# google-research/multinerf

Hardware: AMD Instinct MI355X
Metric: train_rays_per_sec (higher is better)
Workload: dtype bf16 MFMA inputs / fp32 accumulate, fp32 everywhere else

## Files before the change

### include/mnerf.h

```cpp
#ifndef MNERF_H_
#define MNERF_H_

#include <stdint.h>

#ifdef __cplusplus
extern "C" {
#endif

typedef enum {
  MNR_OK = 0,
  MNR_ERR_INVALID_ARGUMENT = -1,
  MNR_ERR_HIP = -2,
  MNR_ERR_UNSUPPORTED = -3
} mnr_status;

const char* mnr_last_error(void);
int mnr_abi_version(void);
int mnr_device_info(int device, int* cu_count, int* lds_bytes_per_cu, char* arch_name, int arch_name_len);

typedef enum { MNR_RAYDIST_IDENTITY = 0, MNR_RAYDIST_RECIPROCAL = 1, MNR_RAYDIST_PIECEWISE = 2,
               MNR_RAYDIST_LOG = 3, MNR_RAYDIST_EXP = 4, MNR_RAYDIST_SQRT = 5, MNR_RAYDIST_SQUARE = 6 } mnr_raydist;

typedef struct {
  int n_prev;
// ... 59 lines not shown

int mnr_viewdir_enc_fill(int64_t B, int n, const float* viewdirs, int deg_view,
                         uint16_t* dst, int ld, int col0, int col_end, void* stream);

typedef enum { MNR_CAM_PERSPECTIVE = 0, MNR_CAM_FISHEYE = 1 } mnr_camtype;
int mnr_pixels_to_rays(int64_t B, const int32_t* pix_x_int, const int32_t* pix_y_int, const int32_t* cam_idx,
                       int num_cams, const float* pixtocams, const float* camtoworlds, const float* distortion6,
                       const float* pixtocam_ndc, int camtype, float* origins, float* directions, float* viewdirs,
                       float* radii, float* imageplane, void* stream);

int mnr_spherical_rays(int H, int W, const float* camtoworld, float* origins, float* directions, float* viewdirs,
                       float* radii, float* imageplane, void* stream);

int mnr_glo_fill(int64_t B, int n, int G, const float* table, const int32_t* cam_idx, int num_embeddings,
                 uint16_t* dst, int ld, int col0, void* stream);
int mnr_glo_bwd(int64_t B, int n, int G, const float* g_a, const float* g_b, const int32_t* cam_idx,
                int num_embeddings, float* grad_table, void* stream);

typedef struct {
  const uint16_t* A1; int lda1; int K1;
  const uint16_t* A2; int lda2; int K2;
  const uint16_t* Bt; int ldb;
  int64_t M;
  int N;
  const float* bias; int n_bias;
  int relu;
  const uint16_t* mask; int ldmask;
  uint16_t* Cb; int ldcb; int nb;
  float* Cf; int ldcf; int f0; int nf;
  uint8_t* mask_bits_out; int ld_bits_out;
  const uint8_t* mask_bits_in; int ld_bits_in;
  int64_t bits_row_mod;
  int a1_layout; int c_layout;
  const uint16_t* vcol; float* vcol_out; const float* vcol_bias;
  int walk_descending;
  int max_wgs;
} mnr_gemm_nt_args;
#define MNR_LAYOUT_ROWMAJOR 0
#define MNR_LAYOUT_PANEL 1

int mnr_gemm_nt_bf16(const mnr_gemm_nt_args* args, void* stream);

#define MNR_CHAIN_MAX_DEPTH 8
typedef struct {
  int64_t M;
  int W;
  int depth;
  const uint16_t* feat;
  int ld_feat; int K0;
  const uint16_t* Bt[MNR_CHAIN_MAX_DEPTH];
  int ldb[MNR_CHAIN_MAX_DEPTH];
  const float* bias[MNR_CHAIN_MAX_DEPTH];
  const uint16_t* w_head;
  const float* b_head;
  float* head_out;
  uint16_t* acts[MNR_CHAIN_MAX_DEPTH];
  uint8_t* bits[MNR_CHAIN_MAX_DEPTH];
  int skip_layer;
} mnr_mlp_chain_fwd_args;
int mnr_mlp_chain_fwd(const mnr_mlp_chain_fwd_args* args, void* stream);

#define MNR_CHAIN_IPE_GROUP_COLS 192
typedef struct {
  mnr_ipe_cfg cfg;
  int n;
  const float* tdist;
  const float* origins; const float* directions; const float* radii; const float* basis;
} mnr_chain_ipe_args;
int mnr_mlp_chain_fwd_ipe(const mnr_mlp_chain_fwd_args* chain, const mnr_chain_ipe_args* ipe, void* stream);

typedef struct {
  int64_t M; int W; int depth;
  const float* g_head;
  const float* w_head;
  const uint8_t* bits[MNR_CHAIN_MAX_DEPTH];
  const uint16_t* Bw[MNR_CHAIN_MAX_DEPTH];
  int ldb[MNR_CHAIN_MAX_DEPTH];
  uint16_t* dY[MNR_CHAIN_MAX_DEPTH];
  const uint16_t* dY_in;
} mnr_mlp_chain_bwd_args;
int mnr_mlp_chain_bwd(const mnr_mlp_chain_bwd_args* args, void* stream);

typedef struct {
  const uint16_t* A; int lda; int K;
  const uint16_t* B; int ldb; int N;
  int64_t M;
  float* C; int ldc;
  int k_valid, n_valid;
  float* bias_out; int bias_n_valid;
  const uint16_t* gcol; float* gcol_out;
  int a_layout, b_layout;
  int m_interleave, max_wgs;
  const float* rank1_g; const float* rank1_w; const uint8_t* rank1_bits; int ld_rank1_bits;
} mnr_gemm_tn_args;

int mnr_gemm_tn_bf16(const mnr_gemm_tn_args* args, void* stream);

int mnr_colsum_bf16(const uint16_t* X, int ld, int64_t M, int n_valid, float* out, void* stream);

typedef struct {
  int64_t src_off; int rows_in; int cols_out;
  int64_t dst_off; int ld; int row0; int col0; int transpose;
} mnr_pack_desc;
int mnr_pack_weights_bf16(const float* params, const mnr_pack_desc* descs_device, int n_desc,
                          int max_elems, uint16_t* dst, void* stream);

int mnr_scatter_add_f32(const float* src, int ld_src, int row0, int col0, int rows, int cols,
                        float* dst, int ld_dst, void* stream);

int mnr_cast_f32_to_bf16(const float* src, int ld_src, int64_t M, int n, uint16_t* dst, int ld_dst,
                         int col0, void* stream);

int mnr_act_fwd_bf16(int kind, int64_t n, const uint16_t* z, uint16_t* a, void* stream);
int mnr_act_bwd_bf16(int kind, int64_t n, const uint16_t* z, uint16_t* d, void* stream);
int mnr_act_tangent_fwd_bf16(int kind, int64_t n, const uint16_t* z, const uint16_t* U, uint16_t* T, void* stream);
int mnr_act_tangent_bwd_bf16(int kind, int64_t n, const uint16_t* z, const uint16_t* U, uint16_t* G, uint16_t* extra, void* stream);

int mnr_add_noise_bf16(int64_t M, int cols, uint16_t* X, int ld, const float* noise, float scale, void* stream);

int mnr_small_head_bwd(int64_t M, int K, int C, const uint16_t* H, int ldh, const float* g,
                       const float* W, uint16_t* dX, int lddx, int apply_relu_mask,
                       float* dW, float* db,
                       const uint8_t* mask_bits ,
                       int ld_bits, int64_t bits_row_mod,
                       float* scratch ,
                       int64_t scratch_floats, void* stream);

typedef enum { MNR_ACT_SIGMOID = 0, MNR_ACT_SAFE_EXP = 1, MNR_ACT_SOFTPLUS = 2, MNR_ACT_EXP = 3,
               MNR_ACT_RELU = 4 } mnr_act;

typedef struct {
  int n;
  int opaque_background;
  int density_act;
  float density_bias;
  float density_noise_std;
  int has_rgb;
  int rgb_act;
  float rgb_premultiplier, rgb_bias, rgb_padding;
  int bg_mode;
  float bg_value;
} mnr_composite_cfg;

int mnr_composite_fwd(const mnr_composite_cfg* cfg, int64_t B, const float* raw_density,
                      const float* density_noise, const float* raw_rgb, const float* tdist,
                      const float* dirs, const float* bg, const float* exposure_scale,
                      float* density, float* rgb, float* weights, float* rgb_out, float* acc,
                      void* stream);

int mnr_composite_bwd(const mnr_composite_cfg* cfg, int64_t B, const float* raw_density,
                      const float* density_noise, const float* raw_rgb, const float* tdist,
                      const float* dirs, const float* bg, const float* exposure_scale,
                      const float* weights, const float* g_rgb_out, const float* g_weights,
                      float* g_raw_density, uint16_t* g_raw_density_bf16, int ld_bf16,
                      float* g_raw_rgb, float* g_exposure_scale , void* stream);

typedef struct {
  mnr_composite_cfg cfg;
  int64_t B, B_valid;
  const float* raw_density; const float* density_noise; const float* raw_rgb; const float* tdist; const float* dirs;
  const float* bg; const float* exposure_scale; const float* weights;
  const float* g_rgb_out;
  const float* g_weights;
  float* g_raw_density; uint16_t* g_raw_density_bf16; int ld_bf16; float* g_raw_rgb; float* g_exposure_scale;
  int data_loss_type; float charb_padding; float data_loss_mult;
  const float* rgb_out; const float* gt; const float* lossmult; int lm_c; const float* denom; float* data_stats;
  int wloss_mode; float wloss_mult; const float* sdist; int n_ref; const float* t_ref; const float* w_ref; float* wloss_stat;
  float* g_x;
} mnr_level_bwd_args;
int mnr_level_bwd(const mnr_level_bwd_args* args, void* stream);

typedef struct {
  int64_t B, B_valid; int n;
  const float* sdist; const float* near; const float* far; int raydist_fn;
  const float* g_x; const float* raw_density; const float* density_noise; float density_noise_std; float density_bias;
  int density_act; const float* dirs;
  const float* g_t0; const float* g_t1;
  float distortion_mult; const float* weights;
  const float* g_sdist_in;
  float* g_sdist;
} mnr_sdist_bwd_args;
int mnr_sdist_bwd(const mnr_sdist_bwd_args* args, void* stream);

int mnr_exposure_scale(int64_t B, const float* exposure_values, const int32_t* exposure_idx,
                       const float* offsets, float* out, void* stream);
int mnr_exposure_scale_bwd(int64_t B_valid, const float* exposure_values, const int32_t* exposure_idx,
                           const float* g_scale, float* g_offsets, void* stream);

int mnr_render_extras(int64_t B, int n, const float* weights, const float* tdist, const float* t_far,
                      float* out, void* stream);

typedef struct {
  int T; int lmax;
  const int32_t* m; const int32_t* l;
  const float* sigma;
  const float* mat;
} mnr_ide_tables;

#define MNR_REF_PRED_NORMALS    1
#define MNR_REF_DENSITY_NORMALS 2
#define MNR_REF_REFLECT         4
#define MNR_REF_IDE             8
#define MNR_REF_N_DOT_V        16
#define MNR_REF_ROUGHNESS      32

int mnr_ref_head_fwd(int64_t M, int n, const float* small, const float* raw_grad, const float* viewdirs,
                     const mnr_ide_tables* tabs, int features, int deg_view, float roughness_bias, uint16_t* vi, int ldvi,
                     int col0, int col_end, float* normals_out, float* normals_pred_out, float* roughness_out, void* stream);
int mnr_ref_head_bwd(int64_t M, int n, const float* small, const float* raw_grad, const float* viewdirs,
                     const mnr_ide_tables* tabs, int features, int deg_view, float roughness_bias, const uint16_t* dvi_a,
                     const uint16_t* dvi_b, int lddvi, int col0, const float* g_npred, const float* g_n,
                     uint16_t* dhb, int lddhb, int col_gp, int col_rough, float* g_raw_grad, void* stream);
int mnr_add_cols_bf16(int64_t M, int cols, const uint16_t* a, int lda, const uint16_t* b, int ldb, uint16_t* dst,
                      int lddst, void* stream);
int mnr_ref_color_fwd(int64_t M, const float* raw_rgb, const float* small, float rgb_premultiplier, float rgb_bias,
                      float rgb_padding, int use_tint, float* rgb_out, void* stream);
int mnr_ref_color_bwd(int64_t M, const float* raw_rgb, const float* small, float rgb_premultiplier, float rgb_bias,
                      float rgb_padding, int use_tint, const float* g_rgb, float* g_raw_rgb, uint16_t* dhb,
                      int lddhb, int col_diffuse, int col_tint, void* stream);
int mnr_ref_losses(int64_t B_valid, int n, float mult_orientation, float mult_pred_normal, int target_is_pred,
                   const float* weights, const float* normals, const float* normals_pred, const float* viewdirs,
                   float* stats, float* g_weights, float* g_normals, float* g_normals_pred, void* stream);
int mnr_density_normals_fwd(int64_t M, const float* raw_grad, float* normals_out, void* stream);
int mnr_density_normals_bwd(int64_t M, const float* raw_grad, const float* g_normals, float* g_raw_grad, void* stream);
int mnr_pred_normals_fwd(int64_t M, const float* small, int ld, int col, float* normals_pred_out, void* stream);
int mnr_pred_normals_bwd(int64_t M, const float* small, int ld, int col, const float* g_normals_pred, uint16_t* dhb, int lddhb,
                         int col_g, void* stream);
int mnr_weighted_sum(int64_t B, int n, int C, const float* weights, const float* values, float* out, void* stream);

typedef enum { MNR_LOSS_MSE = 0, MNR_LOSS_CHARB = 1, MNR_LOSS_RAWNERF = 2 } mnr_data_loss_type;

int mnr_lossmult_sum(int64_t B_valid, const float* lossmult, int lm_c, float* out, void* stream);

int mnr_render_metrics(int64_t B_valid, const float* distance_mean, const float* disps, const float* acc,
                       const float* alphas, const float* normals, const float* normals_gt, float* out_disp,
                       float* out_normal, void* stream);

int mnr_data_loss(int loss_type, float charb_padding, float loss_mult, int64_t B, int64_t B_valid,
                  const float* rgb, const float* gt, const float* lossmult, int lm_c,
                  const float* denom, float* stats, float* g_rgb, void* stream);

int mnr_interlevel_loss(float mult, int64_t B, int64_t B_valid, int n, const float* t, const float* w,
                        int ne, const float* t_env, const float* w_env, float* stats, float* g_w_env,
                        void* stream);

int mnr_distortion_loss(float mult, int64_t B, int64_t B_valid, int n, const float* t, const float* w,
                        float* stats, float* g_w, void* stream);

int mnr_lossfun_outer(int64_t B, int n, const float* t, const float* w, int ne, const float* t_env,
                      const float* w_env, float* out, void* stream);
int mnr_lossfun_distortion(int64_t B, int n, const float* t, const float* w, float* out, void* stream);
// ... 123 lines not shown
```

### multinerf_amd/_lib.py

```python

import ctypes as C
import os
import re

HERE = os.path.dirname(os.path.abspath(__file__))
LIB_PATH = os.environ.get('MNR_LIB_PATH') or os.path.join(HERE, 'libmnerf_hip.so')
LIB_F32_PATH = os.path.join(HERE, 'libmnerf_hip_f32.so')
HEADER_PATH = os.path.join(os.path.dirname(HERE), 'include', 'mnerf.h')
F32_ABSENT = ('mnr_mlp_chain_fwd', 'mnr_mlp_chain_fwd_ipe', 'mnr_mlp_chain_bwd')


def describe():
  stamp = LIB_PATH + '.stamp'
  digest = None
  if os.path.exists(stamp):
    with open(stamp) as f:
      digest = f.read().strip()
  return {'path': os.path.relpath(LIB_PATH, os.path.dirname(HERE)), 'overridden': bool(os.environ.get('MNR_LIB_PATH')),
          'source_digest': digest, 'extra_hipcc_flags': os.environ.get('MNR_EXTRA_HIPCC_FLAGS', '')}

MNR_OK = 0
MNR_ERR_INVALID_ARGUMENT = -1

RAYDIST = {None: 0, 'identity': 0, 'reciprocal': 1, 'piecewise': 2, 'log': 3, 'exp': 4, 'sqrt': 5,
           'square': 6}
ACT = {'sigmoid': 0, 'safe_exp': 1, 'softplus': 2, 'exp': 3, 'relu': 4, 'identity': 5}
DATA_LOSS = {'mse': 0, 'charb': 1, 'rawnerf': 2}
NET_ACT = {'softplus': 1, 'silu': 2}

c_f32p = C.POINTER(C.c_float)
c_u16p = C.POINTER(C.c_uint16)
c_i32p = C.POINTER(C.c_int32)
vp = C.c_void_p


class ResampleCfg(C.Structure):
  _fields_ = [('n_prev', C.c_int), ('n_samples', C.c_int), ('use_dilation', C.c_int),
              ('dilation', C.c_float), ('domain_lo', C.c_float), ('domain_hi', C.c_float),
              ('anneal', C.c_float), ('resample_padding', C.c_float), ('single_jitter', C.c_int),
              ('max_jitter', C.c_float), ('raydist_fn', C.c_int)]


class IpeCfg(C.Structure):
  _fields_ = [('ray_shape', C.c_int), ('warp_contract', C.c_int), ('disable_integration', C.c_int),
              ('basis_k', C.c_int), ('min_deg', C.c_int), ('max_deg', C.c_int)]


class GemmNTArgs(C.Structure):
  _fields_ = [('A1', vp), ('lda1', C.c_int), ('K1', C.c_int),
              ('A2', vp), ('lda2', C.c_int), ('K2', C.c_int),
              ('Bt', vp), ('ldb', C.c_int),
              ('M', C.c_int64), ('N', C.c_int),
              ('bias', vp), ('n_bias', C.c_int), ('relu', C.c_int),
              ('mask', vp), ('ldmask', C.c_int),
              ('Cb', vp), ('ldcb', C.c_int), ('nb', C.c_int),
              ('Cf', vp), ('ldcf', C.c_int), ('f0', C.c_int), ('nf', C.c_int),
              ('mask_bits_out', vp), ('ld_bits_out', C.c_int),
              ('mask_bits_in', vp), ('ld_bits_in', C.c_int),
              ('bits_row_mod', C.c_int64), ('a1_layout', C.c_int), ('c_layout', C.c_int),
              ('vcol', vp), ('vcol_out', vp), ('vcol_bias', vp), ('walk_descending', C.c_int), ('max_wgs', C.c_int)]


class GemmTNArgs(C.Structure):
  _fields_ = [('A', vp), ('lda', C.c_int), ('K', C.c_int),
              ('B', vp), ('ldb', C.c_int), ('N', C.c_int),
              ('M', C.c_int64), ('C', vp), ('ldc', C.c_int),
              ('k_valid', C.c_int), ('n_valid', C.c_int),
              ('bias_out', vp), ('bias_n_valid', C.c_int), ('gcol', vp), ('gcol_out', vp),
              ('a_layout', C.c_int), ('b_layout', C.c_int), ('m_interleave', C.c_int), ('max_wgs', C.c_int),
              ('rank1_g', vp), ('rank1_w', vp), ('rank1_bits', vp), ('ld_rank1_bits', C.c_int)]


CHAIN_MAX_DEPTH = 8


class MlpChainFwdArgs(C.Structure):
  _fields_ = [('M', C.c_int64), ('W', C.c_int), ('depth', C.c_int),
              ('feat', vp), ('ld_feat', C.c_int), ('K0', C.c_int),
              ('Bt', vp * CHAIN_MAX_DEPTH), ('ldb', C.c_int * CHAIN_MAX_DEPTH), ('bias', vp * CHAIN_MAX_DEPTH),
              ('w_head', vp), ('b_head', vp), ('head_out', vp),
              ('acts', vp * CHAIN_MAX_DEPTH), ('bits', vp * CHAIN_MAX_DEPTH), ('skip_layer', C.c_int)]


CHAIN_IPE_GROUP_COLS = 192


class ChainIpeArgs(C.Structure):
  _fields_ = [('cfg', IpeCfg), ('n', C.c_int), ('tdist', vp), ('origins', vp), ('directions', vp), ('radii', vp),
              ('basis', vp)]


class MlpChainBwdArgs(C.Structure):
  _fields_ = [('M', C.c_int64), ('W', C.c_int), ('depth', C.c_int),
              ('g_head', vp), ('w_head', vp),
              ('bits', vp * CHAIN_MAX_DEPTH), ('Bw', vp * CHAIN_MAX_DEPTH), ('ldb', C.c_int * CHAIN_MAX_DEPTH),
              ('dY', vp * CHAIN_MAX_DEPTH), ('dY_in', vp)]


class PackDesc(C.Structure):
  _fields_ = [('src_off', C.c_int64), ('rows_in', C.c_int), ('cols_out', C.c_int),
              ('dst_off', C.c_int64), ('ld', C.c_int), ('row0', C.c_int), ('col0', C.c_int),
              ('transpose', C.c_int)]


class CompositeCfg(C.Structure):
  _fields_ = [('n', C.c_int), ('opaque_background', C.c_int), ('density_act', C.c_int),
              ('density_bias', C.c_float), ('density_noise_std', C.c_float), ('has_rgb', C.c_int),
              ('rgb_act', C.c_int), ('rgb_premultiplier', C.c_float), ('rgb_bias', C.c_float),
              ('rgb_padding', C.c_float), ('bg_mode', C.c_int), ('bg_value', C.c_float)]


class LevelBwdArgs(C.Structure):
  _fields_ = [('cfg', CompositeCfg), ('B', C.c_int64), ('B_valid', C.c_int64),
              ('raw_density', vp), ('density_noise', vp), ('raw_rgb', vp), ('tdist', vp), ('dirs', vp),
              ('bg', vp), ('exposure_scale', vp), ('weights', vp), ('g_rgb_out', vp), ('g_weights', vp),
              ('g_raw_density', vp), ('g_raw_density_bf16', vp), ('ld_bf16', C.c_int), ('g_raw_rgb', vp),
              ('g_exposure_scale', vp),
              ('data_loss_type', C.c_int), ('charb_padding', C.c_float), ('data_loss_mult', C.c_float),
              ('rgb_out', vp), ('gt', vp), ('lossmult', vp), ('lm_c', C.c_int), ('denom', vp), ('data_stats', vp),
              ('wloss_mode', C.c_int), ('wloss_mult', C.c_float), ('sdist', vp), ('n_ref', C.c_int), ('t_ref', vp),
              ('w_ref', vp), ('wloss_stat', vp), ('g_x', vp)]


class SdistBwdArgs(C.Structure):
  _fields_ = [('B', C.c_int64), ('B_valid', C.c_int64), ('n', C.c_int),
              ('sdist', vp), ('near', vp), ('far', vp), ('raydist_fn', C.c_int),
              ('g_x', vp), ('raw_density', vp), ('density_noise', vp), ('density_noise_std', C.c_float),
              ('density_bias', C.c_float), ('density_act', C.c_int), ('dirs', vp),
              ('g_t0', vp), ('g_t1', vp), ('distortion_mult', C.c_float), ('weights', vp),
              ('g_sdist_in', vp), ('g_sdist', vp)]


class IdeTables(C.Structure):
  _fields_ = [('T', C.c_int), ('lmax', C.c_int), ('m', vp), ('l', vp), ('sigma', vp), ('mat', vp)]


class RobustArgs(C.Structure):
  _fields_ = [('B', C.c_int64), ('B_valid', C.c_int64),
              ('patch_size', C.c_int), ('inner_patch_size', C.c_int), ('filter_size', C.c_int), ('enable', C.c_int),
              ('smoothed_inlier_quantile', C.c_double), ('inner_patch_inlier_quantile', C.c_double),
              ('rgb', vp), ('gt', vp), ('lossmult', vp), ('lm_c', C.c_int), ('loss_threshold', vp), ('denom', vp),
              ('mask', vp), ('lossmult_out', vp), ('err', vp), ('stats', vp), ('mse', vp)]


SSIM_MAX_FILTER = 11
CC_FEATURES, CC_GRAM_OUT = 10, 65


class SsimArgs(C.Structure):
  _fields_ = [('H', C.c_int), ('W', C.c_int), ('C', C.c_int), ('crop', C.c_int), ('filter_size', C.c_int),
              ('filter_sigma', C.c_double), ('max_val', C.c_double), ('k1', C.c_double), ('k2', C.c_double),
              ('a', vp), ('b', vp), ('map', vp), ('partials', vp), ('out', vp)]


class SqdiffArgs(C.Structure):
  _fields_ = [('H', C.c_int), ('W', C.c_int), ('C', C.c_int), ('crop', C.c_int), ('quantize', C.c_int),
              ('a_f64', C.c_int), ('b_f64', C.c_int), ('a', vp), ('b', vp), ('q_out', vp), ('partials', vp), ('out', vp)]


class CcGramArgs(C.Structure):
  _fields_ = [('N', C.c_int64), ('eps', C.c_double), ('img', vp), ('ref', vp), ('mask0', vp), ('write_mask0', C.c_int),
              ('partials', vp), ('out', vp)]


VIS_MAX_PERCENTILES = 4
VIS_CURVE = {None: 0, 'identity': 0, 'log': 1, 'neg_log': 2, 'ln': 3}
VIS_PREOP = {None: 0, 'none': 0, 'half': 1, 'tanh': 2, 'coord_mod': 3}


class VisCmapArgs(C.Structure):
  _fields_ = [('H', C.c_int), ('W', C.c_int), ('C', C.c_int), ('value', vp), ('lohi', vp), ('curve', C.c_int),
              ('modulus', C.c_double), ('lut', vp), ('n_lut', C.c_int), ('acc', vp), ('dark', C.c_float), ('light', C.c_float),
              ('width', C.c_int), ('out', vp), ('out_u8', vp)]


class VisMatteArgs(C.Structure):
  _fields_ = [('H', C.c_int), ('W', C.c_int), ('C', C.c_int), ('preop', C.c_int), ('x', vp), ('acc', vp), ('origins', vp),
              ('directions', vp), ('distance', vp), ('dark', C.c_float), ('light', C.c_float), ('width', C.c_int), ('out', vp)]


class AdamCfg(C.Structure):
  _fields_ = [('lr', C.c_float), ('b1', C.c_float), ('b2', C.c_float), ('eps', C.c_float),
              ('bias_corr1', C.c_float), ('bias_corr2', C.c_float), ('grad_max_val', C.c_float),
              ('grad_max_norm', C.c_float)]


i64, i32, f32 = C.c_int64, C.c_int, C.c_float
_PROTOS = {
    'mnr_abi_version': ([], i32),
    'mnr_device_info': ([i32, C.POINTER(i32), C.POINTER(i32), C.c_char_p, i32], i32),
    'mnr_resample_level': ([C.POINTER(ResampleCfg), i64, vp, vp, vp, vp, vp, vp, vp, vp, vp, vp], i32),
    'mnr_resample_level_bwd': ([C.POINTER(ResampleCfg), i64, vp, vp, vp, vp, vp, vp, vp, vp], i32),
    'mnr_sorted_interp': ([i64, i32, i32, vp, vp, vp, vp, vp, vp], i32),
    'mnr_max_dilate_weights': ([i64, i32, vp, vp, f32, f32, f32, vp, vp, vp, vp], i32),
    'mnr_cast_rays_ipe': ([C.POINTER(IpeCfg), i64, i32, vp, vp, vp, vp, vp, vp, i32, vp, vp, vp], i32),
    'mnr_cast_rays_ipe_f32': ([C.POINTER(IpeCfg), i64, i32, vp, vp, vp, vp, vp, vp, vp], i32),
    'mnr_cast_rays_ipe_tangent': ([C.POINTER(IpeCfg), i64, i32, vp, vp, vp, vp, vp, vp, i32, vp], i32),
    'mnr_cast_rays_ipe_bwd': ([C.POINTER(IpeCfg), i64, i32, vp, vp, vp, vp, vp, vp, vp, i32, vp, vp, vp], i32),
    'mnr_cast_rays_ipe_tangent_bwd': ([C.POINTER(IpeCfg), i64, i32, vp, vp, vp, vp, vp, vp, vp, i32, vp, vp, vp], i32),
    'mnr_sdist_bwd': ([C.POINTER(SdistBwdArgs), vp], i32),
    'mnr_viewdir_enc_fill': ([i64, i32, vp, i32, vp, i32, i32, i32, vp], i32),
    'mnr_pixels_to_rays': ([i64, vp, vp, vp, i32, vp, vp, vp, vp, i32, vp, vp, vp, vp, vp, vp], i32),
    'mnr_spherical_rays': ([i32, i32, vp, vp, vp, vp, vp, vp, vp], i32),
    'mnr_glo_fill': ([i64, i32, i32, vp, vp, i32, vp, i32, i32, vp], i32),
    'mnr_glo_bwd': ([i64, i32, i32, vp, vp, vp, i32, vp, vp], i32),
    'mnr_gemm_nt_bf16': ([C.POINTER(GemmNTArgs), vp], i32),
    'mnr_gemm_tn_bf16': ([C.POINTER(GemmTNArgs), vp], i32),
    'mnr_mlp_chain_fwd': ([C.POINTER(MlpChainFwdArgs), vp], i32),
    'mnr_mlp_chain_bwd': ([C.POINTER(MlpChainBwdArgs), vp], i32),
    'mnr_mlp_chain_fwd_ipe': ([C.POINTER(MlpChainFwdArgs), C.POINTER(ChainIpeArgs), vp], i32),
    'mnr_colsum_bf16': ([vp, i32, i64, i32, vp, vp], i32),
    'mnr_pack_weights_bf16': ([vp, vp, i32, i32, vp, vp], i32),
    'mnr_scatter_add_f32': ([vp, i32, i32, i32, i32, i32, vp, i32, vp], i32),
    'mnr_act_fwd_bf16': ([i32, i64, vp, vp, vp], i32),
    'mnr_act_bwd_bf16': ([i32, i64, vp, vp, vp], i32),
    'mnr_act_tangent_fwd_bf16': ([i32, i64, vp, vp, vp, vp], i32),
    'mnr_act_tangent_bwd_bf16': ([i32, i64, vp, vp, vp, vp, vp], i32),
    'mnr_add_noise_bf16': ([i64, i32, vp, i32, vp, f32, vp], i32),
    'mnr_cast_f32_to_bf16': ([vp, i32, i64, i32, vp, i32, i32, vp], i32),
    'mnr_small_head_bwd': ([i64, i32, i32, vp, i32, vp, vp, vp, i32, i32, vp, vp, vp, i32, i64, vp, i64, vp], i32),
    'mnr_composite_fwd': ([C.POINTER(CompositeCfg), i64, vp, vp, vp, vp, vp, vp, vp, vp, vp, vp, vp, vp, vp], i32),
    'mnr_composite_bwd': ([C.POINTER(CompositeCfg), i64, vp, vp, vp, vp, vp, vp, vp, vp, vp, vp, vp, vp, i32,
                           vp, vp, vp], i32),
    'mnr_level_bwd': ([C.POINTER(LevelBwdArgs), vp], i32),
    'mnr_exposure_scale': ([i64, vp, vp, vp, vp, vp], i32),
    'mnr_exposure_scale_bwd': ([i64, vp, vp, vp, vp, vp], i32),
    'mnr_render_extras': ([i64, i32, vp, vp, vp, vp, vp], i32),
    'mnr_ref_head_fwd': ([i64, i32, vp, vp, vp, C.POINTER(IdeTables), i32, i32, f32, vp, i32, i32, i32, vp, vp, vp, vp], i32),
    'mnr_ref_head_bwd': ([i64, i32, vp, vp, vp, C.POINTER(IdeTables), i32, i32, f32, vp, vp, i32, i32, vp, vp, vp, i32, i32, i32, vp, vp],
                         i32),
    'mnr_add_cols_bf16': ([i64, i32, vp, i32, vp, i32, vp, i32, vp], i32),
    'mnr_ref_color_fwd': ([i64, vp, vp, f32, f32, f32, i32, vp, vp], i32),
    'mnr_ref_color_bwd': ([i64, vp, vp, f32, f32, f32, i32, vp, vp, vp, i32, i32, i32, vp], i32),
    'mnr_ref_losses': ([i64, i32, f32, f32, i32, vp, vp, vp, vp, vp, vp, vp, vp, vp], i32),
    'mnr_weighted_sum': ([i64, i32, i32, vp, vp, vp, vp], i32),
    'mnr_density_normals_fwd': ([i64, vp, vp, vp], i32),
    'mnr_density_normals_bwd': ([i64, vp, vp, vp, vp], i32),
    'mnr_pred_normals_fwd': ([i64, vp, i32, i32, vp, vp], i32),
    'mnr_pred_normals_bwd': ([i64, vp, i32, i32, vp, vp, i32, i32, vp], i32),
    'mnr_lossmult_sum': ([i64, vp, i32, vp, vp], i32),
    'mnr_render_metrics': ([i64, vp, vp, vp, vp, vp, vp, vp, vp, vp], i32),
    'mnr_data_loss': ([i32, f32, f32, i64, i64, vp, vp, vp, i32, vp, vp, vp, vp], i32),
    'mnr_interlevel_loss': ([f32, i64, i64, i32, vp, vp, i32, vp, vp, vp, vp, vp], i32),
    'mnr_distortion_loss': ([f32, i64, i64, i32, vp, vp, vp, vp, vp], i32),
    'mnr_lossfun_outer': ([i64, i32, vp, vp, i32, vp, vp, vp, vp], i32),
    'mnr_lossfun_distortion': ([i64, i32, vp, vp, vp, vp], i32),
    'mnr_robustnerf_mask': ([C.POINTER(RobustArgs), vp], i32),
    'mnr_quantile': ([i64, vp, C.c_double, vp, vp], i32),
    'mnr_ssim_partials': ([i32, i32, i32, i32, i32], i32),
    'mnr_ssim': ([C.POINTER(SsimArgs), vp], i32),
    'mnr_image_sqdiff_partials': ([i64], i32),
    'mnr_image_sqdiff': ([C.POINTER(SqdiffArgs), vp], i32),
    'mnr_cc_gram_partials': ([i64], i32),
    'mnr_cc_gram': ([C.POINTER(CcGramArgs), vp], i32),
    'mnr_cc_apply': ([i64, vp, C.POINTER(C.c_double), vp, vp], i32),
    'mnr_weighted_percentile_partials': ([i64], i32),
    'mnr_weighted_percentile': ([i64, vp, vp, i64, vp, i32, C.POINTER(C.c_double), vp, vp, vp], i32),
    'mnr_vis_cmap': ([C.POINTER(VisCmapArgs), vp], i32),
    'mnr_vis_matte': ([C.POINTER(VisMatteArgs), vp], i32),
    'mnr_weight_decay': ([vp, i64, i64, f32, vp, vp, vp, vp], i32),
    'mnr_grad_sqnorm': ([vp, i64, i64, f32, vp, vp], i32),
    'mnr_clip_adam': ([C.POINTER(AdamCfg), i64, i64, vp, vp, vp, vp, vp, vp], i32),
}

_DEBUG_PROTOS = {
    'mnr_debug_gemm_timeline': ([vp], i32),
    'mnr_gemm_nt_set_persistent': ([i32], i32),
    'mnr_level_bwd_set_quad': ([i32], i32),
    'mnr_gemm_nt_set_pipelined': ([i32], i32),
    'mnr_gemm_nt_set_wres': ([i32], i32),
    'mnr_gemm_nt_panel_set_max_wgs': ([i32], i32),
    'mnr_debug_chain_timeline': ([vp], i32),
    'mnr_mlp_chain_set_deferred': ([i32], i32),
    'mnr_mlp_chain_set_max_wgs': ([i32], i32),
}

_lib = None


def header_symbols(path=None):
  with open(path or HEADER_PATH) as f:
    text = f.read()
  text = re.sub(r'/\*.*?\*/', '', text, flags=re.S)
  return sorted(set(re.findall(r'\b(mnr_[a-z0-9_]+)\s*\(', text)))


def _bind(path, absent=()):
  if not os.path.exists(path):
    raise RuntimeError(
        f'{path} is missing: the HIP extension has not been built. Run '
        '`python -m multinerf_amd.build` (needs hipcc, ROCm >= 7.0). There is no CPU fallback.')
  import torch
# ... 69 lines not shown
```

### multinerf_amd/csrc/common.h

```cpp
#pragma once

#include <hip/hip_runtime.h>
#include <stdint.h>
#include <stdlib.h>

#include "../../include/mnerf.h"
#include "../../include/mnerf_debug.h"

#ifdef MNR_DENSE_F32
typedef float bf16;
#else
typedef __bf16 bf16;
#endif
typedef bf16 bf16x2 __attribute__((ext_vector_type(2)));
typedef bf16 bf16x4 __attribute__((ext_vector_type(4)));
typedef bf16 bf16x8 __attribute__((ext_vector_type(8)));
typedef float f32x2 __attribute__((ext_vector_type(2)));
typedef float f32x4 __attribute__((ext_vector_type(4)));
typedef float f32x16 __attribute__((ext_vector_type(16)));
typedef short s16x4 __attribute__((ext_vector_type(4)));

#define MNR_F32_EPS 1.1920928955078125e-07f
#define MNR_F32_MAX 3.4028234663852886e+38f

#define MNR_GLOBAL_PTR(p) ((const __attribute__((address_space(1))) void*)(p))
#define MNR_LDS_PTR(p) ((__attribute__((address_space(3))) void*)(p))

#ifndef MNR_GPU_ONLY
#define MNR_GPU_ONLY(...) __VA_ARGS__
#define MNR_SIM_HOOK(...)
#endif

void mnr_set_error(const char* fmt, ...);

#define MNR_CHECK_ARG(cond, ...)                 \
  do {                                           \
    if (!(cond)) {                               \
      mnr_set_error(__VA_ARGS__);                \
      return MNR_ERR_INVALID_ARGUMENT;           \
    }                                            \
  } while (0)

#define MNR_CHECK_LAUNCH()                                                   \
  do {                                                                       \
    hipError_t e_ = hipGetLastError();                                       \
    if (e_ != hipSuccess) {                                                  \
      mnr_set_error("%s:%d: HIP launch failed: %s", __FILE__, __LINE__,      \
                    hipGetErrorString(e_));                                  \
      return MNR_ERR_HIP;                                                    \
    }                                                                        \
  } while (0)

static inline int mnr_cdiv(long long a, long long b) { return (int)((a + b - 1) / b); }

static inline int mnr_cu_count() {
  static int cus = 0;
  if (cus == 0) {
    hipDeviceProp_t prop;
    int dev = 0;
    (void)hipGetDevice(&dev);
    cus = (hipGetDeviceProperties(&prop, dev) == hipSuccess && prop.multiProcessorCount > 0) ? prop.multiProcessorCount : 256;
  }
  return cus;
}

static inline long long mnr_ray_wave_target() { return 4ll * mnr_cu_count(); }

static inline bool mnr_attr_needed(unsigned long long* mask) {
  int dev = 0;
  (void)hipGetDevice(&dev);
  const unsigned long long bit = 1ull << (dev & 63);
  if (*mask & bit) return false;
  *mask |= bit;
  return true;
}

__device__ __forceinline__ float mnr_nan0_clip01(float x) {
  if (x != x) return 0.0f;
  return fminf(fmaxf(x, 0.0f), 1.0f);
}

__device__ __forceinline__ unsigned mnr_relu_mask_byte(unsigned w0, unsigned w1, unsigned w2, unsigned w3) {
  typedef short mnr_s16x2 __attribute__((ext_vector_type(2)));
  const unsigned w[4] = {w0, w1, w2, w3};
  unsigned m[4];
#pragma unroll
  for (int d = 0; d < 4; ++d) {
    const mnr_s16x2 z = {0, 0};
    const unsigned pos = __builtin_bit_cast(unsigned, __builtin_elementwise_max(__builtin_bit_cast(mnr_s16x2, w[d]), z));
    MNR_GPU_ONLY(asm("v_pk_min_u16 %0, %1, %2" : "=v"(m[d]) : "v"(pos), "v"(0x00010001u)));
    MNR_SIM_HOOK(m[d] = ((pos & 0xffffu) ? 1u : 0u) | ((pos >> 16) ? 0x10000u : 0u));
  }
  const unsigned t = (((m[3] << 2) | m[2]) << 4) | ((m[1] << 2) | m[0]);
  return ((t >> 15) & 0xaau) | (t & 0x55u);
}

__device__ __forceinline__ void nt_wait_lgkmcnt0() { MNR_GPU_ONLY(asm volatile("s_waitcnt lgkmcnt(0)" ::: "memory")); }

__device__ __forceinline__ int mnr_opaque(int v) {
  MNR_GPU_ONLY(asm volatile("" : "+v"(v)));
  return v;
}

__device__ __forceinline__ int mnr_lane_id() {
#ifdef MNR_HIPSIM
  return (int)threadIdx.x & 63;
#else
  return (int)__builtin_amdgcn_mbcnt_hi(~0u, __builtin_amdgcn_mbcnt_lo(~0u, (unsigned)mnr_opaque(0)));
#endif
}
__device__ __forceinline__ int mnr_opaque_s(int v) {
  MNR_GPU_ONLY(asm volatile("" : "+s"(v)));
  return v;
}
__device__ __forceinline__ void nt_launder(bf16x8& f) { MNR_GPU_ONLY(asm volatile("" : "+v"(f))); }

template <int N>
__device__ __forceinline__ void nt_wait_vmcnt() {
  MNR_GPU_ONLY(asm volatile("s_waitcnt vmcnt(%0)" ::"n"(N) : "memory"));
  MNR_SIM_HOOK(hipsim::wait_vmcnt(N));
}

__device__ __forceinline__ float mnr_softplus(float x) {
  return fmaxf(x, 0.0f) + log1pf(expf(-fabsf(x)));
}

__device__ __forceinline__ float mnr_sigmoid(float x) { return 1.0f / (1.0f + expf(-x)); }
```

### multinerf_amd/csrc/fused_mlp.hip

```cpp
#include <stdio.h>

#include <type_traits>

#include "common.h"

#define FM_ROWS 256
#define FM_KT_BYTES 32768

__device__ __forceinline__ int fm_opaque(int v) {
  MNR_GPU_ONLY(asm volatile("" : "+v"(v)));
  return v;
}

__device__ __forceinline__ int fm_off(int row, int slot) { return row * 128 + ((slot ^ ((row >> 1) & 7)) << 4); }

template <int ROWS>
__device__ __forceinline__ void fm_stage_tile(const bf16* __restrict__ tile_base, int ld, char* lds_tile, int wave, int lane) {
#pragma unroll
  for (int i = 0; i < ROWS * 8 / 512; ++i) {
    const int cbase = (i * 8 + wave) * 64;
    const int c = cbase + lane;
    const int r = c >> 3;
    const int slot = (c & 7) ^ ((r >> 1) & 7);
    const bf16* src = tile_base + (unsigned)(r * ld + slot * 8);
// ... 335 lines not shown
    __syncthreads();
    {
      const bf16* Bt0 = (const bf16*)p.Bt[0];
      const bf16* feat_tile = feat + m0 * (int64_t)p.ld_feat;
      auto stage = [&](int kt) {
        char* base = smem + (kt & 1) * C::STAGE_BYTES;
        const int ln = fm_opaque(lane);
        fm_stage_tile<FM_ROWS>(feat_tile + kt * 64, p.ld_feat, base, wave, ln);
        fm_stage_tile<W>(Bt0 + kt * 64, p.ldb[0], base + FM_KT_BYTES, wave, ln);
      };
      constexpr int HB = C::RB > 4 ? 4 : C::RB;
      constexpr int NH = C::RB / HB;
      const int ln0 = fm_opaque(lane), frow = ln0 & 31, khalf = ln0 >> 5;
      const int sw = (frow >> 1) & 7;
      stage(0);
      for (int kt = 0; kt < nk0; ++kt) {
        MNR_GPU_ONLY(asm volatile("s_waitcnt vmcnt(0)" ::: "memory"));
        MNR_SIM_HOOK(hipsim::wait_vmcnt(0));
        __builtin_amdgcn_s_barrier();
        asm volatile("" ::: "memory");
        if (kt + 1 < nk0) stage(kt + 1);
        const char* As = smem + (kt & 1) * C::STAGE_BYTES + (rg * C::RB * 32 + frow) * 128;
        const char* Ws = smem + (kt & 1) * C::STAGE_BYTES + FM_KT_BYTES + (cw * 32 + frow) * 128;
        bf16x8 wf[4];
#pragma unroll
        for (int ks = 0; ks < 4; ++ks) wf[ks] = *(const bf16x8*)(Ws + (((ks * 2 + khalf) ^ sw) << 4));
        bf16x8 fa[2][HB];
        auto read_batch = [&](int step, bf16x8 (&f)[HB]) {
          const int ks = step / NH, h = step % NH;
          const char* base = As + h * HB * 4096 + (((ks * 2 + khalf) ^ sw) << 4);
#pragma unroll
          for (int i = 0; i < HB; ++i) f[i] = *(const bf16x8*)(base + i * 4096);
        };
        read_batch(0, fa[0]);
        __builtin_amdgcn_sched_group_barrier(0x100, 4 + HB, 0);
#pragma unroll
        for (int step = 0; step < 4 * NH; ++step) {
          const int ks = step / NH, h = step % NH;
          if (step + 1 < 4 * NH) {
            read_batch(step + 1, fa[(step + 1) & 1]);
            __builtin_amdgcn_sched_group_barrier(0x100, HB, 0);
          }
#pragma unroll
          for (int i = 0; i < HB; ++i)
            acc[h * HB + i] = __builtin_amdgcn_mfma_f32_32x32x16_bf16(wf[ks], fa[step & 1][i], acc[h * HB + i], 0, 0, 0);
          __builtin_amdgcn_sched_group_barrier(0x008, HB, 0);
        }
      }
    }

    FM_STAMP(1);
    bf16x8 w0[FM_WCHUNK];
    if (p.depth > 1) {
      const int ln = fm_opaque(lane);
      fm_load_wchunk((const bf16*)p.Bt[1], p.ldb[1], cw, ln & 31, ln >> 5, 0, w0);
    }
    for (int li = 0; li < p.depth; ++li) {
      if (li > 0) {
        if (defer) fm_layer_mfma_defer<W>(smem, (const bf16*)p.Bt[li], p.ldb[li], cw, rg, lane, w0, acc, tid, m0, (bf16*)p.acts[li - 1], p.bits[li - 1]);
        else fm_layer_mfma<W, 0>(smem, (const bf16*)p.Bt[li], p.ldb[li], cw, rg, lane, w0, acc);
        if (li == p.skip_layer)
          fm_skip_segment<W>(smem + C::SKIP_OFF, feat + m0 * (int64_t)p.ld_feat, p.ld_feat, p.K0, (const bf16*)p.Bt[li],
                             p.ldb[li], W, cw, rg, wave, lane, acc);
        if (li + 1 < p.depth) {
          const int ln = fm_opaque(lane);
          fm_load_wchunk((const bf16*)p.Bt[li + 1], p.ldb[li + 1], cw, ln & 31, ln >> 5, 0, w0);
        }
      }
      FM_STAMP(2 + 3 * li);
      fm_lds_barrier();
      fm_epilogue<W, false>(smem, cw, rg, lane, acc, (const float*)(smem + C::BIAS_OFF) + li * W, no_bits);
      fm_lds_barrier();
      FM_STAMP(3 + 3 * li);
      const bool last = li == p.depth - 1;
      if (last || !defer)
        fm_copy_out_dispatch<W>(smem, tid, m0, (bf16*)p.acts[li], p.bits[li], last ? (const bf16*)p.w_head : nullptr, b_head,
                                p.head_out);
      FM_STAMP(4 + 3 * li);
    }
    if (tl_on) g_fm_timeline[32 * (int64_t)blockIdx.x + 31] = __builtin_amdgcn_s_memrealtime();
  }
}

template <int W>
__global__ __launch_bounds__(512) void mlp_chain_bwd_kernel(mnr_mlp_chain_bwd_args p, int defer) {
  typedef FmCfg<W> C;
  extern __shared__ __attribute__((aligned(16))) char smem[];
  const int tid = threadIdx.x, lane = tid & 63;
  const int wave = __builtin_amdgcn_readfirstlane(tid >> 6);
  const int cw = wave % C::NW, rg = wave / C::NW;
  const int64_t tiles = p.M / FM_ROWS;

  for (int64_t tile = blockIdx.x; tile < tiles; tile += gridDim.x) {
    const int64_t m0 = tile * FM_ROWS;
    const bool tl_on = g_fm_timeline != nullptr && tid == 0 && tile == (int64_t)blockIdx.x + gridDim.x;
    FM_STAMP(0);
    if (tl_on) g_fm_timeline[32 * (int64_t)blockIdx.x + 30] = __builtin_amdgcn_s_memrealtime();
    __syncthreads();
    if (p.dY_in) {
      const bf16* src = (const bf16*)p.dY_in + m0 * (int64_t)W;
      const int ln = fm_opaque(lane);
#pragma unroll
      for (int kt = 0; kt < C::NKT; ++kt) fm_stage_tile<FM_ROWS>(src + kt * 64, W, smem + kt * FM_KT_BYTES, wave, ln);
      MNR_GPU_ONLY(asm volatile("s_waitcnt vmcnt(0)" ::: "memory"));
      MNR_SIM_HOOK(hipsim::wait_vmcnt(0));
    } else {
      const int last = p.depth - 1;
      const int t_ = fm_opaque(tid);
      const int row0 = t_ / C::CPR, ch = t_ % C::CPR;
      float wh[8];
      {
        const f32x4 a = *(const f32x4*)(p.w_head + ch * 8), b = *(const f32x4*)(p.w_head + ch * 8 + 4);
#pragma unroll
        for (int e = 0; e < 4; ++e) wh[e] = a[e], wh[4 + e] = b[e];
      }
      char* lptr = smem + (ch >> 3) * FM_KT_BYTES + row0 * 128 + (((ch & 7) ^ ((row0 >> 1) & 7)) << 4);
      const int64_t ro = m0 + row0;
      const uint8_t* bl = p.bits[last] + ro * (W / 8) + (ch & ~3);
      const float* gp = p.g_head + ro;
      bf16* dst = p.dY[last] ? (bf16*)p.dY[last] + ro * W + ch * 8 : nullptr;
      float g[C::COPY_ITERS];
      unsigned mb[C::COPY_ITERS];
#pragma unroll
      for (int u = 0; u < C::COPY_ITERS; ++u) {
        g[u] = gp[u * C::ROW_STEP];
        mb[u] = *(const unsigned*)(bl + (int64_t)u * C::ROW_STEP * (W / 8)) >> ((ch & 3) * 8);
      }
#pragma unroll
      for (int u = 0; u < C::COPY_ITERS; ++u) {
        bf16x8 v;
#pragma unroll
        for (int e = 0; e < 8; ++e) v[e] = (bf16)(((mb[u] >> e) & 1u) ? g[u] * wh[e] : 0.0f);
        *(bf16x8*)(lptr + u * C::ROW_STEP * 128) = v;
        if (dst) *(bf16x8*)(dst + (int64_t)u * C::ROW_STEP * W) = v;
      }
    }
    bf16x8 w0[FM_WCHUNK];
    if (p.depth > 1) {
      const int ln = fm_opaque(lane);
      fm_load_wchunk((const bf16*)p.Bw[p.depth - 1], p.ldb[p.depth - 1], cw, ln & 31, ln >> 5, 0, w0);
    }
    __syncthreads();
    FM_STAMP(1);
    for (int li = p.depth - 1; li >= 1; --li) {
      unsigned mbits[C::RB];
      {
        const int frow = fm_opaque(lane) & 31;
        const uint8_t* bl = p.bits[li - 1] + (m0 + rg * C::RB * 32) * (int64_t)(W / 8) + cw * 4 + (unsigned)(frow * (W / 8));
#pragma unroll
        for (int rb = 0; rb < C::RB; ++rb) mbits[rb] = *(const unsigned*)(bl + (int64_t)rb * 32 * (W / 8));
      }
      f32x16 acc[C::RB];
      if (defer && li < p.depth - 1) fm_layer_mfma<W, 1>(smem, (const bf16*)p.Bw[li], p.ldb[li], cw, rg, lane, w0, acc, tid, m0, (bf16*)p.dY[li], nullptr);
      else fm_layer_mfma<W, 0>(smem, (const bf16*)p.Bw[li], p.ldb[li], cw, rg, lane, w0, acc);
      FM_STAMP(2 + 3 * li);
      if (li > 1) {
        const int ln = fm_opaque(lane);
        fm_load_wchunk((const bf16*)p.Bw[li - 1], p.ldb[li - 1], cw, ln & 31, ln >> 5, 0, w0);
      }
      fm_lds_barrier();
      fm_epilogue<W, true>(smem, cw, rg, lane, acc, nullptr, mbits);
      fm_lds_barrier();
      FM_STAMP(3 + 3 * li);
      if (!defer || li == 1) fm_copy_out<W, true, false, false>(smem, tid, m0, (bf16*)p.dY[li - 1], nullptr, nullptr, 0.0f, nullptr);
      FM_STAMP(4 + 3 * li);
    }
    if (tl_on) g_fm_timeline[32 * (int64_t)blockIdx.x + 31] = __builtin_amdgcn_s_memrealtime();
  }
}

static int g_fm_defer = 1;
extern "C" int mnr_mlp_chain_set_deferred(int on) {
  g_fm_defer = on;
  return MNR_OK;
}

static int g_fm_max_wgs = 0;
extern "C" int mnr_mlp_chain_set_max_wgs(int n) {
  g_fm_max_wgs = n > 0 ? n : 0;
  return MNR_OK;
}

static int fm_grid(int64_t tiles) {
  int cus = mnr_cu_count();
  if (g_fm_max_wgs > 0 && g_fm_max_wgs < cus) cus = g_fm_max_wgs;
  return (int)(tiles < cus ? tiles : cus);
}

static int fm_check_common(const char* who, int64_t M, int W, int depth) {
  MNR_CHECK_ARG(M > 0 && M % FM_ROWS == 0, "%s: M=%lld must be a positive multiple of 256", who, (long long)M);
  MNR_CHECK_ARG(W == 128 || W == 256, "%s: width %d is not 128 or 256", who, W);
  MNR_CHECK_ARG(depth >= 1 && depth <= MNR_CHAIN_MAX_DEPTH, "%s: depth %d out of range", who, depth);
  return MNR_OK;
}

extern "C" int mnr_mlp_chain_fwd(const mnr_mlp_chain_fwd_args* a, void* stream) {
  MNR_CHECK_ARG(a != nullptr, "mnr_mlp_chain_fwd: null args");
  if (int s = fm_check_common("mnr_mlp_chain_fwd", a->M, a->W, a->depth)) return s;
  MNR_CHECK_ARG(a->feat && a->K0 > 0 && a->K0 % 64 == 0 && a->ld_feat % 8 == 0 && a->ld_feat >= a->K0 && a->ld_feat <= (1 << 20),
                "mnr_mlp_chain_fwd: feature matrix needs K0 %% 64 == 0 and ld_feat %% 8 == 0");
  for (int i = 0; i < a->depth; ++i) {
    MNR_CHECK_ARG(a->Bt[i] && a->bias[i] && a->ldb[i] % 8 == 0 && a->ldb[i] >= (i == 0 ? a->K0 : a->W),
                  "mnr_mlp_chain_fwd: layer %d operand", i);
    MNR_CHECK_ARG(((uintptr_t)a->bias[i] % 16) == 0, "mnr_mlp_chain_fwd: bias[%d] must be 16-byte aligned", i);
    MNR_CHECK_ARG(((uintptr_t)a->Bt[i] % 16) == 0 && (!a->acts[i] || ((uintptr_t)a->acts[i] % 16) == 0) &&
                      (!a->bits[i] || ((uintptr_t)a->bits[i] % 4) == 0),
                  "mnr_mlp_chain_fwd: layer %d pointers must be 16-byte (bits: 4-byte) aligned", i);
  }
  MNR_CHECK_ARG(((uintptr_t)a->feat % 16) == 0, "mnr_mlp_chain_fwd: feat must be 16-byte aligned");
  MNR_CHECK_ARG(!a->w_head || (a->head_out && ((uintptr_t)a->w_head % 16) == 0), "mnr_mlp_chain_fwd: head needs head_out");
  MNR_CHECK_ARG(a->skip_layer <= 0 || (a->skip_layer < a->depth && a->K0 % 16 == 0 && a->ldb[a->skip_layer] >= a->W + a->K0),
                "mnr_mlp_chain_fwd: skip_layer %d needs 0 < skip_layer < depth and an operand of W + K0 columns", a->skip_layer);
  const int grid = fm_grid(a->M / FM_ROWS);
  if (a->W == 256) {
    (void)hipFuncSetAttribute((const void*)mlp_chain_fwd_kernel<256>, hipFuncAttributeMaxDynamicSharedMemorySize, FmCfg<256>::LDS_BYTES);
    hipLaunchKernelGGL(mlp_chain_fwd_kernel<256>, dim3(grid), dim3(512), FmCfg<256>::LDS_BYTES, (hipStream_t)stream, *a, g_fm_defer);
  } else {
    (void)hipFuncSetAttribute((const void*)mlp_chain_fwd_kernel<128>, hipFuncAttributeMaxDynamicSharedMemorySize, FmCfg<128>::LDS_BYTES);
    hipLaunchKernelGGL(mlp_chain_fwd_kernel<128>, dim3(grid), dim3(512), FmCfg<128>::LDS_BYTES, (hipStream_t)stream, *a, g_fm_defer);
  }
  MNR_CHECK_LAUNCH();
  return MNR_OK;
}

extern "C" int mnr_mlp_chain_bwd(const mnr_mlp_chain_bwd_args* a, void* stream) {
  MNR_CHECK_ARG(a != nullptr, "mnr_mlp_chain_bwd: null args");
  if (int s = fm_check_common("mnr_mlp_chain_bwd", a->M, a->W, a->depth)) return s;
  MNR_CHECK_ARG(a->dY_in ? ((uintptr_t)a->dY_in % 16) == 0 : (a->g_head && a->w_head && ((uintptr_t)a->w_head % 16) == 0),
                "mnr_mlp_chain_bwd: needs dY_in (16-byte aligned) or a head gradient with a 16-byte-aligned head kernel");
  for (int i = 0; i < a->depth; ++i) {
    MNR_CHECK_ARG(a->bits[i] && ((uintptr_t)a->bits[i] % 4) == 0, "mnr_mlp_chain_bwd: layer %d needs its ReLU mask bits", i);
    MNR_CHECK_ARG(a->dY[i] || i == a->depth - 1, "mnr_mlp_chain_bwd: dY[%d] missing", i);
    MNR_CHECK_ARG(!(a->dY_in && i == a->depth - 1 && a->dY[i]), "mnr_mlp_chain_bwd: with dY_in the last dY is the input itself");
    MNR_CHECK_ARG(!a->dY[i] || ((uintptr_t)a->dY[i] % 16) == 0, "mnr_mlp_chain_bwd: dY[%d] must be 16-byte aligned", i);
    if (i >= 1)
      MNR_CHECK_ARG(a->Bw[i] && a->ldb[i] % 8 == 0 && a->ldb[i] >= a->W && ((uintptr_t)a->Bw[i] % 16) == 0,
                    "mnr_mlp_chain_bwd: layer %d operand", i);
  }
  const int grid = fm_grid(a->M / FM_ROWS);
  if (a->W == 256) {
    (void)hipFuncSetAttribute((const void*)mlp_chain_bwd_kernel<256>, hipFuncAttributeMaxDynamicSharedMemorySize, FmCfg<256>::LDS_BYTES);
    hipLaunchKernelGGL(mlp_chain_bwd_kernel<256>, dim3(grid), dim3(512), FmCfg<256>::LDS_BYTES, (hipStream_t)stream, *a, g_fm_defer);
  } else {
    (void)hipFuncSetAttribute((const void*)mlp_chain_bwd_kernel<128>, hipFuncAttributeMaxDynamicSharedMemorySize, FmCfg<128>::LDS_BYTES);
    hipLaunchKernelGGL(mlp_chain_bwd_kernel<128>, dim3(grid), dim3(512), FmCfg<128>::LDS_BYTES, (hipStream_t)stream, *a, g_fm_defer);
  }
  MNR_CHECK_LAUNCH();
  return MNR_OK;
}

#pragma clang fp contract(off)
#include "ipe_math.h"

#define FM_IPE_MAX_KS (MNR_CHAIN_IPE_GROUP_COLS / 16)
#define FM_IPE_MAX_K 24

template <int W>
struct FmIpeCfg {
  typedef FmCfg<W> C;
  static constexpr int GROUP_BYTES = 3 * FM_KT_BYTES;
  static constexpr int MAIN = C::X_BYTES > GROUP_BYTES ? C::X_BYTES : GROUP_BYTES;
  static constexpr int BIAS_OFF = MAIN;
  static constexpr int GS_OFF = BIAS_OFF + MNR_CHAIN_MAX_DEPTH * W * 4;
  static constexpr int BASIS_OFF = GS_OFF + FM_ROWS * (int)sizeof(FeSample);
  static constexpr int LDS_BYTES = BASIS_OFF + 3 * FM_IPE_MAX_K * 4;
  static_assert(LDS_BYTES <= 160 * 1024, "LDS");
  static_assert(sizeof(FeSample) % 4 == 0 && GS_OFF % 16 == 0, "alignment");
};

template <int W>
__global__ __launch_bounds__(512) void mlp_chain_fwd_ipe_kernel(mnr_mlp_chain_fwd_args p, mnr_chain_ipe_args q) {
  typedef FmCfg<W> C;
  typedef FmIpeCfg<W> I;
  extern __shared__ __attribute__((aligned(16))) char smem[];
  const int tid = threadIdx.x, lane = tid & 63;
  const int wave = __builtin_amdgcn_readfirstlane(tid >> 6);
  const int cw = wave % C::NW, rg = wave / C::NW;
  const int64_t tiles = p.M / FM_ROWS;
  const int K = q.cfg.basis_k;
  const int ngroups = (q.cfg.max_deg - q.cfg.min_deg) / 4;
  const int pad_slots = MNR_CHAIN_IPE_GROUP_COLS / 8 - K;
  const unsigned no_bits[C::RB] = {};
  const float b_head = (p.w_head && p.b_head) ? p.b_head[0] : 0.0f;
  FeSample* gs = (FeSample*)(smem + I::GS_OFF);
  float* bs = (float*)(smem + I::BASIS_OFF);
  for (int i = tid; i < p.depth * W; i += 512) ((float*)(smem + I::BIAS_OFF))[i] = p.bias[i / W][i % W];
  for (int i = tid; i < K * 3; i += 512) bs[i] = q.basis[i];
  const bf16* Bt0 = (const bf16*)p.Bt[0];
  const int rpi = 512 / K;

  for (int64_t tile = blockIdx.x; tile < tiles; tile += gridDim.x) {
    const int64_t m0 = tile * FM_ROWS;
    const bool tl_on = g_fm_timeline != nullptr && tid == 0 && tile == (int64_t)blockIdx.x + gridDim.x;
    FM_STAMP(0);
    if (tl_on) g_fm_timeline[32 * (int64_t)blockIdx.x + 30] = __builtin_amdgcn_s_memrealtime();
    __syncthreads();
    if (tid < FM_ROWS) {
      const int64_t s = m0 + tid;
      const int64_t ray = s / q.n;
      const int j = (int)(s - ray * q.n);
      const float t0 = q.tdist[ray * (q.n + 1) + j], t1 = q.tdist[ray * (q.n + 1) + j + 1];
      float o[3], d[3];
#pragma unroll
      for (int i = 0; i < 3; ++i) {
        o[i] = q.origins[ray * 3 + i];
        d[i] = q.directions[ray * 3 + i];
      }
      FeSample g;
      fe_gaussian(q.cfg, t0, t1, o, d, q.radii[ray], g);
      gs[tid] = g;
    }
    for (int e = tid; e < FM_ROWS * pad_slots; e += 512) {
      const int r = e / pad_slots, sl = K + e % pad_slots;
      const u32x4 z = {0u, 0u, 0u, 0u};
      *(u32x4*)(smem + (sl >> 3) * FM_KT_BYTES + fm_off(r, sl & 7)) = z;
    }
    f32x16 acc[C::RB];
#pragma unroll
    for (int rb = 0; rb < C::RB; ++rb)
#pragma unroll
      for (int r = 0; r < 16; ++r) acc[rb][r] = 0.0f;
    __syncthreads();

    auto encode = [&](int g, int r_lo, int r_hi) {
      const float sc0 = ldexpf(1.0f, q.cfg.min_deg + 4 * g);
      const int et = fm_opaque(tid);
      const int er0 = et / K, ek = et - er0 * K;
      if (et < rpi * K) {
        const float px = bs[ek * 3 + 0], py = bs[ek * 3 + 1], pz = bs[ek * 3 + 2];
        unsigned cb[8];
#pragma unroll
// ... 127 lines not shown
```

### multinerf_amd/csrc/gemm.hip

```cpp
#include <stdio.h>
#include <stdlib.h>
#include <type_traits>

#include "common.h"

#ifdef MNR_DENSE_F32
#include "dense_f32.inc"
#else


#define NT_CPAD 16

template <int MI_, int NJ_, int WM_, int WN_, int EPI_BATCH_ = 0, int BIAS_LDS_ = 0, int PIPE_ = 0, int DBG_ = 0, int BK_ = 64, int STAGES_ = 2>
struct NtCfg {
  static constexpr int DBG = DBG_;
  static constexpr bool PIPE = PIPE_ != 0;
  static constexpr int EPI_BATCH = EPI_BATCH_;
  static constexpr int MI = MI_, NJ = NJ_, WM = WM_, WN = WN_, BK = BK_, STAGES = STAGES_;
  static constexpr int MINW = 1;
  static constexpr int BM = 32 * MI * WM, BN = 32 * NJ * WN;
  static constexpr int THREADS = 64 * WM * WN;
  static constexpr int ROWB = BK * 2;
  static constexpr int SLOTS = ROWB / 16;
  static constexpr int A_BYTES = BM * ROWB, B_BYTES = BN * ROWB;
// ... 814 lines not shown
      float gc[U][4];
      unsigned mb[U];
#pragma unroll
      for (int u = 0; u < U; ++u) {
        const int64_t r = min(rb + (int64_t)u * row_lanes, r1 - 1);
        h[u] = *(const bf16x8*)(H + r * ldh + cg * 8);
#pragma unroll
        for (int c = 0; c < 4; ++c) gc[u][c] = (c < C) ? g[r * C + c] : 0.0f;
        mb[u] = 0xffu;
        if (mbits) mb[u] = mbits[(bits_row_mod > 0 ? r % bits_row_mod : r) * ld_bits + cg];
      }
#pragma unroll
      for (int u = 0; u < U; ++u) {
        const int64_t r = rb + (int64_t)u * row_lanes;
        if (r >= r1) {
#pragma unroll
          for (int c = 0; c < 4; ++c) gc[u][c] = 0.0f;
        }
#pragma unroll
        for (int c = 0; c < 4; ++c) sb[c] += gc[u][c];
        bf16x8 o;
#pragma unroll
        for (int e = 0; e < 8; ++e) {
          const float hv = (float)h[u][e];
          float gx = 0.0f;
#pragma unroll
          for (int c = 0; c < 4; ++c) {
            gx += gc[u][c] * w[e][c];
            aw[e][c] += hv * gc[u][c];
          }
          o[e] = (bf16)(((relu_mask && !(hv > 0.0f)) || !((mb[u] >> e) & 1u)) ? 0.0f : gx);
        }
        if (dX && r < r1) *(bf16x8*)(dX + r * lddx + cg * 8) = o;
      }
    }
  }
  if (dW) {
    for (int c = 0; c < C; ++c) {
      __syncthreads();
#pragma unroll
      for (int e = 0; e < 8; ++e) red[threadIdx.x * 8 + e] = aw[e][c];
      __syncthreads();
      if (rl == 0) {
#pragma unroll
        for (int e = 0; e < 8; ++e) {
          float sum = 0.0f;
          for (int k2 = 0; k2 < row_lanes; ++k2) sum += red[(k2 * groups + cg) * 8 + e];
          if (partials) partials[(int64_t)blockIdx.x * (K * C + C) + (cg * 8 + e) * C + c] = sum;
          else unsafeAtomicAdd(dW + (int64_t)(cg * 8 + e) * C + c, sum);
        }
      }
    }
  }
  if (partials && db) {
    __syncthreads();
    if (cg == 0 && rl < row_lanes)
      for (int c = 0; c < C; ++c) red[rl * 4 + c] = sb[c];
    __syncthreads();
    if (threadIdx.x < C) {
      float sum = 0.0f;
      for (int k2 = 0; k2 < row_lanes; ++k2) sum += red[k2 * 4 + threadIdx.x];
      partials[(int64_t)blockIdx.x * (K * C + C) + K * C + threadIdx.x] = sum;
    }
  } else if (db && cg == 0 && rl < row_lanes) {
    for (int c = 0; c < C; ++c) unsafeAtomicAdd(db + c, sb[c]);
  }
}

__global__ void small_head_reduce_kernel(int nblk, int n, int n_dw, const float* __restrict__ partials, float* dW,
                                         float* db) {
  const int i = blockIdx.x * blockDim.x + threadIdx.x;
  if (i >= n) return;
  const int per = (nblk + gridDim.y - 1) / gridDim.y;
  const int b0 = blockIdx.y * per, b1 = min(nblk, b0 + per);
  float sum = 0.0f;
  for (int b = b0; b < b1; ++b) sum += partials[(int64_t)b * n + i];
  if (i < n_dw) {
    if (dW) unsafeAtomicAdd(dW + i, sum);
  } else if (db) {
    unsafeAtomicAdd(db + (i - n_dw), sum);
  }
}

extern "C" int mnr_small_head_bwd(int64_t M, int K, int C, const uint16_t* H, int ldh, const float* g,
                                  const float* W, uint16_t* dX, int lddx, int apply_relu_mask, float* dW,
                                  float* db, const uint8_t* mask_bits, int ld_bits, int64_t bits_row_mod,
                                  float* scratch, int64_t scratch_floats, void* stream) {
  MNR_CHECK_ARG(M > 0 && K > 0 && C >= 1 && C <= 4 && H && g && W, "mnr_small_head_bwd: bad arguments (1 <= C <= 4)");
  MNR_CHECK_ARG(K % 8 == 0 && K / 8 <= 256 && ldh % 8 == 0 && (!dX || lddx % 8 == 0),
                "mnr_small_head_bwd: K must be a multiple of 8 (<= 2048) and the pitches multiples of 8");
  int rows_auto = (int)(((M + 511) / 512 + 63) / 64 * 64);
  if (rows_auto < 512) rows_auto = 512;
  int rows_per_block = rows_auto;
  float* partials = nullptr;
  if (scratch && dW) {
    constexpr int blocks_env = 512;
    int rows_p = (int)(((M + blocks_env - 1) / blocks_env + 63) / 64 * 64);
    if (rows_p < 256) rows_p = 256;
    if ((int64_t)mnr_cdiv(M, rows_p) * (K * C + C) <= scratch_floats) {
      rows_per_block = rows_p;
      partials = scratch;
    }
  }
  const int grid = mnr_cdiv(M, rows_per_block);
  hipLaunchKernelGGL(small_head_bwd_kernel<4>, dim3(grid), dim3(256), 0, (hipStream_t)stream, M, K, C, (const bf16*)H, ldh, g, W,
                     (bf16*)dX, lddx, apply_relu_mask, dW, db, rows_per_block, mask_bits, ld_bits, bits_row_mod, partials);
  MNR_CHECK_LAUNCH();
  if (partials) {
    const int n = K * C + C;
    hipLaunchKernelGGL(small_head_reduce_kernel, dim3(mnr_cdiv(n, 128), 16), dim3(128), 0, (hipStream_t)stream, grid, n,
                       K * C, partials, dW, db);
    MNR_CHECK_LAUNCH();
  }
  return MNR_OK;
}
```

### multinerf_amd/csrc/render.hip

```cpp
#include "common.h"
#include "ray_losses.h"

#define CP_THREADS 64

__device__ __forceinline__ float cp_act(int kind, float x) {
  switch (kind) {
    case MNR_ACT_SIGMOID: return mnr_sigmoid(x);
    case MNR_ACT_SAFE_EXP: return expf(fminf(x, 88.0f));
    case MNR_ACT_SOFTPLUS: return mnr_softplus(x);
    case MNR_ACT_EXP: return expf(x);
    case MNR_ACT_RELU: return fmaxf(x, 0.0f);
    default: return x;
  }
}

__device__ __forceinline__ float cp_act_grad(int kind, float x, float y) {
  switch (kind) {
    case MNR_ACT_SIGMOID: return y * (1.0f - y);
    case MNR_ACT_SAFE_EXP: return y;
    case MNR_ACT_SOFTPLUS: return mnr_sigmoid(x);
    case MNR_ACT_EXP: return y;
    case MNR_ACT_RELU: return x > 0.0f ? 1.0f : 0.0f;
    default: return 1.0f;
  }
// ... 225 lines not shown
    } else if (a.wloss_mode == 2 && valid) {
      const float scale = a.wloss_mult / (float)a.B_valid;
      for (int i = 0; i < n; ++i) {
        const float ui = (l_s[(i + 1) * S + r] + l_s[i * S + r]) / 2.0f, wi = l_w[i * S + r];
        float inner = 0.0f;
        for (int j = 0; j < n; ++j) inner += l_w[j * S + r] * fabsf(ui - (l_s[(j + 1) * S + r] + l_s[j * S + r]) / 2.0f);
        const float dt = l_s[(i + 1) * S + r] - l_s[i * S + r];
        s_wloss += wi * inner + wi * wi * dt / 3.0f;
        l_gw[i * S + r] += scale * (2.0f * inner + (2.0f / 3.0f) * wi * dt);
      }
    }
    const float dx = a.dirs[ray * 3], dy = a.dirs[ray * 3 + 1], dz = a.dirs[ray * 3 + 2];
    const float dnorm = sqrtf(dx * dx + dy * dy + dz * dz);
    float ex[3] = {1.0f, 1.0f, 1.0f};
    if (a.exposure_scale) { ex[0] = a.exposure_scale[ray * 3]; ex[1] = a.exposure_scale[ray * 3 + 1]; ex[2] = a.exposure_scale[ray * 3 + 2]; }
    float b[3] = {c.bg_value, c.bg_value, c.bg_value};
    if (c.bg_mode == 1) { b[0] = a.bg[ray * 3]; b[1] = a.bg[ray * 3 + 1]; b[2] = a.bg[ray * 3 + 2]; }
    float acc = 0.0f;
    for (int i = 0; i < n; ++i) acc += l_w[i * S + r];
    const float g_bgw = (1.0f - acc > 0.0f) ? (go[0] * b[0] + go[1] * b[1] + go[2] * b[2]) : 0.0f;
    float run = 0.0f;
    for (int i = 0; i + 1 < n; ++i) {
      const float sigma = cp_act(c.density_act, l_den[i * S + r] + c.density_bias);
      run += sigma * (l_t[(i + 1) * S + r] - l_t[i * S + r]) * dnorm;
    }
    float suffix = 0.0f;
    float ges[3] = {0.0f, 0.0f, 0.0f};
    for (int i = n - 1; i >= 0; --i) {
      const float w = l_w[i * S + r];
      const float raw = l_den[i * S + r] + c.density_bias;
      const float sigma = cp_act(c.density_act, raw);
      const float delta = (l_t[(i + 1) * S + r] - l_t[i * S + r]) * dnorm;
      const bool opaque_last = c.opaque_background && i == n - 1;
      const float x = opaque_last ? INFINITY : sigma * delta;
      const float t_next = expf(-(run + x));
      float ghat = l_gw[i * S + r] - g_bgw;
      float gc[3] = {0.0f, 0.0f, 0.0f};
      if (c.has_rgb) {
#pragma unroll
        for (int ch = 0; ch < 3; ++ch) {
          const float z = c.rgb_premultiplier * l_rgb[(3 * i + ch) * S + r] + c.rgb_bias;
          const float y = cp_act(c.rgb_act, z);
          const float col_pre = y * (1.0f + 2.0f * c.rgb_padding) - c.rgb_padding;
          const float col = col_pre * ex[ch];
          ghat += go[ch] * col;
          ges[ch] += w * go[ch] * col_pre;
          gc[ch] = w * go[ch] * ex[ch] * (1.0f + 2.0f * c.rgb_padding) * cp_act_grad(c.rgb_act, z, y) *
                   c.rgb_premultiplier;
        }
#pragma unroll
        for (int ch = 0; ch < 3; ++ch) l_rgb[(3 * i + ch) * S + r] = gc[ch];
      }
      float gx = ghat * t_next - suffix;
      if (opaque_last) gx = 0.0f;
      suffix += ghat * w;
      l_den[i * S + r] = gx * delta * cp_act_grad(c.density_act, raw, sigma);
      l_gw[i * S + r] = gx;
      if (i > 0) {
        const float sp = cp_act(c.density_act, l_den[(i - 1) * S + r] + c.density_bias);
        run -= sp * (l_t[i * S + r] - l_t[(i - 1) * S + r]) * dnorm;
      }
    }
    if (a.g_exposure_scale) {
#pragma unroll
      for (int ch = 0; ch < 3; ++ch) a.g_exposure_scale[ray * 3 + ch] += ges[ch];
    }
  }
  if (a.data_loss_type >= 0 && a.data_stats) {
    s_mse = ls_wave_sum(s_mse);
    s_dloss = ls_wave_sum(s_dloss);
    if (threadIdx.x == 0) {
      const float denom = *a.denom;
      unsafeAtomicAdd(a.data_stats + 0, s_mse / denom);
      unsafeAtomicAdd(a.data_stats + 1, a.data_loss_mult * s_dloss / denom);
    }
  }
  if (a.wloss_mode != 0 && a.wloss_stat) {
    s_wloss = ls_wave_sum(s_wloss);
    const float norm = a.wloss_mode == 1 ? (float)a.B_valid * (float)a.n_ref : (float)a.B_valid;
    if (threadIdx.x == 0) unsafeAtomicAdd(a.wloss_stat, a.wloss_mult * s_wloss / norm);
  }
  __syncthreads();
  if (a.g_raw_density) cp_store_rows(l_den, a.g_raw_density + ray0 * n, rows, n, S);
  if (a.g_raw_density_bf16) {
    bf16* gb = (bf16*)a.g_raw_density_bf16;
    for (int e = threadIdx.x; e < rows * n; e += CP_THREADS) {
      const int rr = e / n, i = e % n;
      gb[(ray0 * n + e) * (int64_t)a.ld_bf16] = (bf16)l_den[i * S + rr];
    }
  }
  if (c.has_rgb && a.g_raw_rgb) cp_store_rows(l_rgb, a.g_raw_rgb + ray0 * n * 3, rows, 3 * n, S);
  if (a.g_x) cp_store_rows(l_gw, a.g_x + ray0 * n, rows, n, S);
}

#define LB_LPR 4
#define LB_RPW (CP_THREADS / LB_LPR)

template <int CTRL>
__device__ __forceinline__ float lb_dpp(float v) {
  return __builtin_bit_cast(float, __builtin_amdgcn_update_dpp(0, __builtin_bit_cast(int, v), CTRL, 0xf, 0xf, false));
}
__device__ __forceinline__ float lb_quad_sum(float v) {
  v += lb_dpp<0xB1>(v);
  v += lb_dpp<0x4E>(v);
  return v;
}
__device__ __forceinline__ float lb_quad_prefix(float v, int q) {
  const float a = lb_dpp<0x90>(v);
  if (q >= 1) v += a;
  const float b = lb_dpp<0x40>(v);
  if (q >= 2) v += b;
  return v;
}
__device__ __forceinline__ float lb_quad_suffix(float v, int q) {
  const float a = lb_dpp<0xF9>(v);
  if (q <= 2) v += a;
  const float b = lb_dpp<0xFE>(v);
  if (q <= 1) v += b;
  return v;
}

struct LbLay {
  int den, t, w, rgb, gw, scr, stride;
};
__host__ __device__ inline LbLay lb_layout(int n, int has_rgb, int wloss_mode, int n_ref) {
  LbLay L;
  int o = 0;
  L.den = o; o += n;
  L.t = o; o += n + 1;
  L.w = o; o += n;
  L.rgb = o; o += has_rgb ? 3 * n : 0;
  L.gw = o; o += n;
  L.scr = o;
  int loss = wloss_mode != 0 ? n + 1 : 0;
  if (wloss_mode == 1) loss += (n + 1) + 3 * (n_ref + 1);
  o += loss > 3 * n ? loss : 3 * n;
  o = (o + 3) & ~3;
  if (((o >> 2) & 1) == 0) o += 4;
  L.stride = o;
  return L;
}

__global__ __launch_bounds__(CP_THREADS) void level_bwd_quad_kernel(mnr_level_bwd_args a) {
  extern __shared__ __attribute__((aligned(16))) float lds[];
  const mnr_composite_cfg c = a.cfg;
  const int n = c.n;
  const LbLay L = lb_layout(n, c.has_rgb, a.wloss_mode, a.n_ref);
  const int64_t B = a.B;
  const int64_t ray0 = (int64_t)blockIdx.x * LB_RPW;
  const int rows = (int)min((int64_t)LB_RPW, B - ray0);
  auto load_rows = [&](int off, const float* src, int len) {
    for (int e = threadIdx.x; e < rows * len; e += CP_THREADS) {
      const int rr = e / len, i = e - rr * len;
      lds[rr * L.stride + off + i] = src[e];
    }
  };
  load_rows(L.den, a.raw_density + ray0 * n, n);
  load_rows(L.t, a.tdist + ray0 * (n + 1), n + 1);
  load_rows(L.w, a.weights + ray0 * n, n);
  if (c.has_rgb) load_rows(L.rgb, a.raw_rgb + ray0 * n * 3, 3 * n);
  if (a.g_weights) {
    load_rows(L.gw, a.g_weights + ray0 * n, n);
  } else {
    for (int e = threadIdx.x; e < LB_RPW * n; e += CP_THREADS) lds[(e / n) * L.stride + L.gw + e % n] = 0.0f;
  }
  if (a.wloss_mode != 0) load_rows(L.scr, a.sdist + ray0 * (n + 1), n + 1);
  if (a.density_noise && c.density_noise_std > 0.0f) {
    __syncthreads();
    for (int e = threadIdx.x; e < rows * n; e += CP_THREADS) {
      const int rr = e / n, i = e - rr * n;
      lds[rr * L.stride + L.den + i] += c.density_noise_std * a.density_noise[ray0 * n + e];
// ... 143 lines not shown
  {
    float carry = 0.0f;
    for (int j = 0; j < J; ++j) {
      const int i = 4 * j + q;
      const bool in = i < n;
      const float raw = (in ? l_den[i] : 0.0f) + c.density_bias;
      const float sigma = cp_act(c.density_act, raw);
      const float delta = in ? (l_t[i + 1] - l_t[i]) * dnorm : 0.0f;
      const bool opaque_last = c.opaque_background && i == n - 1;
      const float x = opaque_last ? INFINITY : (in ? sigma * delta : 0.0f);
      const float inc = lb_quad_prefix(x, q);
      const float below = lb_dpp<0x90>(inc);
      const float before = (q == 0 ? 0.0f : below) + carry;
      carry += lb_dpp<0xFF>(inc);
      if (in) {
        const float w = l_w[i];
        l_tn[i] = expf(-(before + x));
        l_dg[i] = delta * cp_act_grad(c.density_act, raw, sigma);
        float ghat = l_gw[i] - g_bgw;
        if (c.has_rgb) {
#pragma unroll
          for (int ch = 0; ch < 3; ++ch) {
            const float z = c.rgb_premultiplier * l_rgb[3 * i + ch] + c.rgb_bias;
            const float y = cp_act(c.rgb_act, z);
            const float col_pre = y * (1.0f + 2.0f * c.rgb_padding) - c.rgb_padding;
            const float col = col_pre * ex[ch];
            ghat += go[ch] * col;
            ges[ch] += w * go[ch] * col_pre;
            l_rgb[3 * i + ch] = w * go[ch] * ex[ch] * (1.0f + 2.0f * c.rgb_padding) * cp_act_grad(c.rgb_act, z, y) *
                                c.rgb_premultiplier;
          }
        }
        l_gh[i] = ghat;
      }
    }
  }
  {
    float carry = 0.0f;
    for (int j = J - 1; j >= 0; --j) {
      const int i = 4 * j + q;
      const bool in = i < n;
      const float ghat = in ? l_gh[i] : 0.0f;
      const float inc = lb_quad_suffix(in ? ghat * l_w[i] : 0.0f, q);
      const float above = lb_dpp<0xF9>(inc);
      const float after = (q == 3 ? 0.0f : above) + carry;
      carry += lb_dpp<0x00>(inc);
      if (in) {
        float gx = ghat * l_tn[i] - after;
        if (c.opaque_background && i == n - 1) gx = 0.0f;
        l_den[i] = gx * l_dg[i];
        l_gh[i] = gx;
      }
    }
  }
  if (a.g_exposure_scale) {
#pragma unroll
    for (int ch = 0; ch < 3; ++ch) {
      const float g = lb_quad_sum(ges[ch]);
      if (live && q == 0) a.g_exposure_scale[ray * 3 + ch] += g;
    }
  }
  if (a.data_loss_type >= 0 && a.data_stats) {
    s_mse = ls_wave_sum(s_mse);
    s_dloss = ls_wave_sum(s_dloss);
    if (threadIdx.x == 0) {
      const float denom = *a.denom;
      unsafeAtomicAdd(a.data_stats + 0, s_mse / denom);
      unsafeAtomicAdd(a.data_stats + 1, a.data_loss_mult * s_dloss / denom);
    }
  }
  if (a.wloss_mode != 0 && a.wloss_stat) {
    s_wloss = ls_wave_sum(s_wloss);
    const float norm = a.wloss_mode == 1 ? (float)a.B_valid * (float)a.n_ref : (float)a.B_valid;
    if (threadIdx.x == 0) unsafeAtomicAdd(a.wloss_stat, a.wloss_mult * s_wloss / norm);
  }
  __syncthreads();
  auto store_rows = [&](int off, float* dst, int len) {
    for (int e = threadIdx.x; e < rows * len; e += CP_THREADS) {
      const int rr = e / len, i = e - rr * len;
      dst[e] = lds[rr * L.stride + off + i];
    }
  };
  if (a.g_raw_density) store_rows(L.den, a.g_raw_density + ray0 * n, n);
  if (a.g_raw_density_bf16) {
    bf16* gb = (bf16*)a.g_raw_density_bf16;
    for (int e = threadIdx.x; e < rows * n; e += CP_THREADS) {
      const int rr = e / n, i = e - rr * n;
      gb[(ray0 * n + e) * (int64_t)a.ld_bf16] = (bf16)lds[rr * L.stride + L.den + i];
    }
  }
  if (c.has_rgb && a.g_raw_rgb) store_rows(L.rgb, a.g_raw_rgb + ray0 * n * 3, 3 * n);
  if (a.g_x) store_rows(L.scr + 2 * n, a.g_x + ray0 * n, n);
}

__global__ __launch_bounds__(CP_THREADS) void composite_fwd_quad_kernel(
    mnr_composite_cfg c, int64_t B, int stride, const float* __restrict__ raw_density, const float* __restrict__ noise,
    const float* __restrict__ raw_rgb, const float* __restrict__ tdist, const float* __restrict__ dirs,
    const float* __restrict__ bg, const float* __restrict__ expo, float* __restrict__ density,
    float* __restrict__ rgb, float* __restrict__ weights, float* __restrict__ rgb_out, float* __restrict__ acc_out) {
  extern __shared__ __attribute__((aligned(16))) float lds[];
  const int n = c.n;
  const int o_den = 0, o_t = n, o_w = 2 * n + 1, o_rgb = 3 * n + 1;
  const int64_t ray0 = (int64_t)blockIdx.x * LB_RPW;
  const int rows = (int)min((int64_t)LB_RPW, B - ray0);
  auto load_rows = [&](int off, const float* src, int len) {
    for (int e = threadIdx.x; e < rows * len; e += CP_THREADS) {
      const int rr = e / len, i = e - rr * len;
      lds[rr * stride + off + i] = src[e];
    }
  };
  auto store_rows = [&](int off, float* dst, int len) {
    for (int e = threadIdx.x; e < rows * len; e += CP_THREADS) {
      const int rr = e / len, i = e - rr * len;
      dst[e] = lds[rr * stride + off + i];
    }
  };
  load_rows(o_den, raw_density + ray0 * n, n);
  load_rows(o_t, tdist + ray0 * (n + 1), n + 1);
  if (c.has_rgb) load_rows(o_rgb, raw_rgb + ray0 * n * 3, 3 * n);
  if (noise && c.density_noise_std > 0.0f) {
    __syncthreads();
    for (int e = threadIdx.x; e < rows * n; e += CP_THREADS) {
      const int rr = e / n, i = e - rr * n;
      lds[rr * stride + o_den + i] += c.density_noise_std * noise[ray0 * n + e];
    }
  }
  __syncthreads();
  const int r = threadIdx.x >> 2, q = threadIdx.x & 3;
  const bool live = r < rows;
  const int64_t ray = live ? ray0 + r : B - 1;
  float* X = lds + r * stride;
  const float dx = dirs[ray * 3], dy = dirs[ray * 3 + 1], dz = dirs[ray * 3 + 2];
  const float dnorm = sqrtf(dx * dx + dy * dy + dz * dz);
  float ex[3] = {1.0f, 1.0f, 1.0f};
  if (expo) { ex[0] = expo[ray * 3]; ex[1] = expo[ray * 3 + 1]; ex[2] = expo[ray * 3 + 2]; }
  float carry = 0.0f, acc = 0.0f, cr = 0.0f, cg = 0.0f, cb = 0.0f;
  const int J = (n + 3) >> 2;
  for (int j = 0; j < J; ++j) {
    const int i = 4 * j + q;
    const bool in = i < n;
    const float sigma = cp_act(c.density_act, (in ? X[o_den + i] : 0.0f) + c.density_bias);
    const float delta = in ? (X[o_t + i + 1] - X[o_t + i]) * dnorm : 0.0f;
    float x = in ? sigma * delta : 0.0f;
    if (c.opaque_background && i == n - 1) x = INFINITY;
    const float inc = lb_quad_prefix(x, q);
    const float below = lb_dpp<0x90>(inc);
    const float before = (q == 0 ? 0.0f : below) + carry;
    carry += lb_dpp<0xFF>(inc);
    if (in) {
      const float w = (1.0f - expf(-x)) * expf(-before);
      X[o_den + i] = sigma;
      X[o_w + i] = w;
      acc += w;
      if (c.has_rgb) {
#pragma unroll
        for (int ch = 0; ch < 3; ++ch) {
          float v = cp_act(c.rgb_act, c.rgb_premultiplier * X[o_rgb + 3 * i + ch] + c.rgb_bias);
          v = v * (1.0f + 2.0f * c.rgb_padding) - c.rgb_padding;
          v *= ex[ch];
          X[o_rgb + 3 * i + ch] = v;
          if (ch == 0) cr += w * v; else if (ch == 1) cg += w * v; else cb += w * v;
        }
      }
    }
  }
  acc = lb_quad_sum(acc);
  cr = lb_quad_sum(cr);
  cg = lb_quad_sum(cg);
  cb = lb_quad_sum(cb);
  if (live && q == 0) {
    const float bgw = fmaxf(0.0f, 1.0f - acc);
    float b0 = c.bg_value, b1 = c.bg_value, b2 = c.bg_value;
    if (c.bg_mode == 1) { b0 = bg[ray * 3]; b1 = bg[ray * 3 + 1]; b2 = bg[ray * 3 + 2]; }
    rgb_out[ray * 3 + 0] = cr + bgw * b0;
    rgb_out[ray * 3 + 1] = cg + bgw * b1;
    rgb_out[ray * 3 + 2] = cb + bgw * b2;
    if (acc_out) acc_out[ray] = acc;
  }
  __syncthreads();
  store_rows(o_den, density + ray0 * n, n);
  store_rows(o_w, weights + ray0 * n, n);
  if (c.has_rgb && rgb) store_rows(o_rgb, rgb + ray0 * n * 3, 3 * n);
}

static size_t lb_floats_per_ray(const mnr_level_bwd_args* a) {
  const int n = a->cfg.n;
  size_t f = (size_t)(6 * n + 1) + n;
  if (a->wloss_mode != 0) f += n + 1;
  if (a->wloss_mode == 1) f += 3 * (size_t)a->n_ref + 2;
  return f;
}

extern "C" int mnr_level_bwd(const mnr_level_bwd_args* a, void* stream) {
  MNR_CHECK_ARG(a != nullptr, "mnr_level_bwd: null args");
  const mnr_composite_cfg* cfg = &a->cfg;
  MNR_CHECK_ARG(a->B > 0 && a->B_valid > 0 && a->B_valid <= a->B && a->raw_density && a->tdist && a->dirs && a->weights,
                "mnr_level_bwd: null argument");
  MNR_CHECK_ARG(cfg->n >= 1 && cfg->n <= 1024, "mnr_level_bwd: n out of range");
  MNR_CHECK_ARG(a->g_raw_density || a->g_raw_density_bf16, "mnr_level_bwd: no density-gradient output");
  MNR_CHECK_ARG(!cfg->has_rgb || a->raw_rgb, "mnr_level_bwd: has_rgb needs raw_rgb");
  MNR_CHECK_ARG(cfg->bg_mode == 0 || a->bg, "mnr_level_bwd: bg_mode 1 needs bg");
  MNR_CHECK_ARG(a->data_loss_type < 0 || (a->data_loss_type <= MNR_LOSS_RAWNERF && a->rgb_out && a->gt && a->lossmult &&
                                          a->denom && (a->lm_c == 1 || a->lm_c == 3)),
                "mnr_level_bwd: the fused data loss needs rgb_out, gt, lossmult [B,1|3] and denom");
  MNR_CHECK_ARG(a->wloss_mode >= 0 && a->wloss_mode <= 2, "mnr_level_bwd: wloss_mode must be 0, 1 or 2");
  MNR_CHECK_ARG(a->wloss_mode == 0 || a->sdist, "mnr_level_bwd: weight losses need this level's sdist");
  MNR_CHECK_ARG(a->wloss_mode != 1 || (a->n_ref >= 1 && a->n_ref <= 1024 && a->t_ref && a->w_ref),
                "mnr_level_bwd: the interlevel loss needs the final level's (t_ref, w_ref)");
  const LbLay lay = lb_layout(cfg->n, cfg->has_rgb, a->wloss_mode, a->n_ref);
  const size_t quad_lds = (size_t)lay.stride * LB_RPW * 4;
  if (g_level_bwd_quad && quad_lds <= quad_lds_max()) {
    static unsigned long long attr_q = 0;
    if (quad_lds > 64 * 1024 && mnr_attr_needed(&attr_q))
      (void)hipFuncSetAttribute((const void*)level_bwd_quad_kernel, hipFuncAttributeMaxDynamicSharedMemorySize, 160 * 1024);
    hipLaunchKernelGGL(level_bwd_quad_kernel, dim3(mnr_cdiv(a->B, LB_RPW)), dim3(CP_THREADS), quad_lds, (hipStream_t)stream, *a);
    MNR_CHECK_LAUNCH();
    return MNR_OK;
  }
  const size_t fpr = lb_floats_per_ray(a);
  int S = CP_THREADS;
  while (S > 1 && fpr * S * 4 > 150 * 1024) S >>= 1;
  while (S > 8 && a->B / S < mnr_ray_wave_target()) S >>= 1;
  const size_t lds = fpr * S * 4;
  MNR_CHECK_ARG(lds <= 160 * 1024, "mnr_level_bwd: n=%d too long for LDS staging", cfg->n);
  static unsigned long long attr_set = 0;
  if (mnr_attr_needed(&attr_set)) {
    (void)hipFuncSetAttribute((const void*)level_bwd_kernel, hipFuncAttributeMaxDynamicSharedMemorySize, 160 * 1024);
  }
  hipLaunchKernelGGL(level_bwd_kernel, dim3(mnr_cdiv(a->B, S)), dim3(CP_THREADS), lds, (hipStream_t)stream, *a, S);
  MNR_CHECK_LAUNCH();
  return MNR_OK;
}

extern "C" int mnr_composite_bwd(const mnr_composite_cfg* cfg, int64_t B, const float* raw_density,
                                 const float* density_noise, const float* raw_rgb, const float* tdist,
                                 const float* dirs, const float* bg, const float* exposure_scale,
                                 const float* weights, const float* g_rgb_out, const float* g_weights,
                                 float* g_raw_density, uint16_t* g_raw_density_bf16, int ld_bf16,
                                 float* g_raw_rgb, float* g_exposure_scale, void* stream) {
  MNR_CHECK_ARG(cfg != nullptr, "mnr_composite_bwd: null cfg");
  mnr_level_bwd_args a = {};
  a.cfg = *cfg;
  a.B = a.B_valid = B;
  a.raw_density = raw_density;
  a.density_noise = density_noise;
  a.raw_rgb = raw_rgb;
  a.tdist = tdist;
  a.dirs = dirs;
  a.bg = bg;
  a.exposure_scale = exposure_scale;
  a.weights = weights;
  a.g_rgb_out = g_rgb_out;
  a.g_weights = g_weights;
  a.g_raw_density = g_raw_density;
  a.g_raw_density_bf16 = g_raw_density_bf16;
  a.ld_bf16 = ld_bf16;
  a.g_raw_rgb = g_raw_rgb;
  a.g_exposure_scale = g_exposure_scale;
  a.data_loss_type = -1;
  a.wloss_mode = 0;
  return mnr_level_bwd(&a, stream);
}


__global__ void render_extras_kernel(int64_t B, int n, const float* __restrict__ weights,
                                     const float* __restrict__ tdist, const float* __restrict__ t_far,
                                     float* __restrict__ out) {
  const int64_t ray = (int64_t)blockIdx.x * blockDim.x + threadIdx.x;
  if (ray >= B) return;
  const float* w = weights + ray * n;
  const float* t = tdist + ray * (n + 1);
  float acc = 0.0f, e = 0.0f;
  for (int i = 0; i < n; ++i) {
    acc += w[i];
    e += w[i] * logf(0.5f * (t[i] + t[i + 1]));
  }
  float dm = expf(e / fmaxf(MNR_F32_EPS, acc));
  if (dm != dm) dm = INFINITY;
  dm = fminf(fmaxf(dm, t[0]), t[n]);
  out[ray * 4 + 0] = dm;
  const float ps[3] = {0.05f, 0.5f, 0.95f};
  const int nb = n + 1;
// ... 180 lines not shown
```

### multinerf_amd/models.py

```python

import ctypes as C
import dataclasses
import math
from typing import Any, Dict, List, Optional, Tuple

import numpy as np
import torch

from multinerf_amd import _lib as L
from multinerf_amd import geopoly
from multinerf_amd import gin
from multinerf_amd import ops
from multinerf_amd import utils

F32_EPS = float(np.finfo(np.float32).eps)
bf16 = torch.bfloat16
f32 = torch.float32


def _rup(x, m):
  return (x + m - 1) // m * m


def _in_library(fn):
  import functools

  @functools.wraps(fn)
  def wrapped(self, *a, **kw):
    with self.library():
      return fn(self, *a, **kw)
  return wrapped


def _rank1_last(plan, D, W, feature_gradient):
  concat_last = bool(plan.trunk[D - 1][1])
  k_in = plan.ldF if D == 1 else W
  return bool(_RANK1_LAST and W % 256 == 0 and k_in % 256 == 0 and not concat_last and not (feature_gradient and D == 1))


_USE_BITS = True
_USE_CHAIN = True
_FUSED_IPE = True
_HEAD_VCOL = True
_HEAD_GCOL = True
_PANEL = True
_MERGE_PROPS = True
_RANK1_LAST = True
_PAIR_DXDW = True
_TANGENT_CHAIN = True
_HEAD_K32 = True




@dataclasses.dataclass
class MLP:
  net_depth: int = 8
  net_width: int = 256
  bottleneck_width: int = 256
  net_depth_viewdirs: int = 1
  net_width_viewdirs: int = 128
  net_activation: str = 'relu'
  min_deg_point: int = 0
  max_deg_point: int = 12
  weight_init: str = 'he_uniform'
  skip_layer: int = 4
  skip_layer_dir: int = 4
  num_rgb_channels: int = 3
  deg_view: int = 4
  use_reflections: bool = False
  use_directional_enc: bool = False
  enable_pred_roughness: bool = False
  roughness_activation: str = 'softplus'
  roughness_bias: float = -1.
  use_diffuse_color: bool = False
  use_specular_tint: bool = False
  use_n_dot_v: bool = False
  bottleneck_noise: float = 0.0
  density_activation: str = 'softplus'
  density_bias: float = -1.
  density_noise: float = 0.
  rgb_premultiplier: float = 1.
  rgb_activation: str = 'sigmoid'
  rgb_bias: float = 0.
  rgb_padding: float = 0.001
  enable_pred_normals: bool = False
  disable_density_normals: bool = False
  disable_rgb: bool = False
  warp_fn: Optional[str] = None
  basis_shape: str = 'icosahedron'
  basis_subdivisions: int = 2

  def setup_checks(self):
    if self.use_reflections and not (self.enable_pred_normals or not self.disable_density_normals):
      raise ValueError('Normals must be computed for reflection directions.')

  def is_ref(self):
    return (not self.disable_rgb) and bool(self.use_reflections or self.use_directional_enc or self.enable_pred_roughness or
                                           self.use_diffuse_color or self.use_specular_tint or self.use_n_dot_v)

  def ref_features(self):
    return ((ops.REF_PRED_NORMALS if self.enable_pred_normals else 0) |
            (0 if self.disable_density_normals else ops.REF_DENSITY_NORMALS) |
            (ops.REF_REFLECT if self.use_reflections else 0) | (ops.REF_IDE if self.use_directional_enc else 0) |
            (ops.REF_N_DOT_V if self.use_n_dot_v else 0) | (ops.REF_ROUGHNESS if self.enable_pred_roughness else 0))

  def hip_supported(self):
    bad = []
    ref_flags = ('enable_pred_normals', 'use_reflections', 'use_directional_enc', 'enable_pred_roughness',
                 'use_diffuse_color', 'use_specular_tint', 'use_n_dot_v')
    on = [f for f in ref_flags if getattr(self, f)]
    if not self.disable_density_normals:
      on.append('density normals')
    if self.use_directional_enc and not self.enable_pred_roughness:
      bad.append('use_directional_enc without enable_pred_roughness (undefined in the reference: ref_utils.py:147)')
    if self.use_directional_enc and not self.use_reflections and not self.disable_rgb:
      bad.append('use_directional_enc without use_reflections (undefined in the reference: ref_utils.py:154)')
    if self.use_n_dot_v and not self.enable_pred_normals and self.disable_density_normals:
      bad.append('use_n_dot_v without normals (undefined in the reference: models.py:560-563)')
    if on and self.disable_rgb:
      bad.append('normals ' + str(on) + ' on a density-only MLP (disable_rgb)')
    if self.enable_pred_roughness and self.roughness_activation != 'softplus':
      bad.append('roughness_activation != softplus')
    if self.is_ref() and not self.use_directional_enc and self.deg_view > 11:
      bad.append('deg_view > 11 in the positional encoding of a per-sample direction')
    if self.net_activation not in ('relu', 'softplus', 'silu'):
      bad.append(f'net_activation={self.net_activation}')
    if self.warp_fn not in (None, 'contract'):
      bad.append(f'warp_fn={self.warp_fn}')
    if self.net_width <= 0:
      bad.append('net_width must be positive')
    if not self.disable_rgb and self.bottleneck_width <= 0:
      bad.append('bottleneck_width must be positive')
# ... 1010 lines not shown

  @_in_library
  def backward_level(self, lv, flat, grads, g_rgb_out, g_weights, g_expo=None, g_normals=None, g_npred=None, losses=None,
                     g_x_out=None, g_feat_out=None, g_tfeat_out=None):
    plan: MLPPlan = lv['plan']
    hp = plan.hp
    M, n, tag = lv['M'], lv['n'], lv['tag']
    R = self._saved['rays']
    mlp = lv['mlp']
    acts = mlp['acts']
    x_last = acts[-1]
    W = plan.W
    D = len(plan.trunk)
    slot = 'nerf' if lv['level'] == self.num_levels - 1 else 'prop'

    def dy_buf(i):
      return self._buf(('bwd', slot, 'dA' if (D - 1 - i) % 2 == 0 else 'dB', W), (M, W), bf16)

    def dv_buf(i, nv):
      return self._buf(('bwd', slot, 'dV0' if (nv - 1 - i) % 2 == 0 else 'dV1', WV), (M, WV), bf16)

    if not mlp.get('chain'):
      dA = dy_buf(D - 1)

    def gslice(off, size):
      return grads[off:off + size]

    relu = hp.net_activation == 'relu'
    panel = bool(mlp.get('panel'))
    PAN = ops.LAYOUT_PANEL
    lay_c = dict(c_layout=PAN) if panel else {}
    lay_ac = dict(a1_layout=PAN, c_layout=PAN) if panel else {}
    tn_a = dict(a_layout=PAN) if panel else {}
    tn_b = dict(b_layout=PAN) if panel else {}

    def act_vjp(z, d):
      if not relu:
        ops.act_bwd(hp.net_activation, z, d)

    def mask_kw(i):
      if not relu:
        return {}
      if mlp['bits'][i] is not None:
        return dict(bits_in=mlp['bits'][i])
      return dict(mask=acts[i], ldmask=W)

    def feat_grad(i, dy, dy_panel=False):
      if g_feat_out is None:
        return
      e_ = plan.packed[('trunk', i)]
      out = self._buf(('bwd', slot, 'g_feat', len(g_feat_out)), (M, plan.ldF), bf16)
      ops.gemm_nt(dy, self._w(plan, e_['bf_off'], plan.ldF, e_['bf_ld']), M=M, N=plan.ldF, K1=e_['bf_ld'], Cb=out,
                  ldcb=plan.ldF, nb=plan.ldF, **(dict(a1_layout=PAN) if dy_panel else {}))
      g_feat_out.append(out)

    g_raw_grad = None
    if plan.has_rgb and not plan.use_viewdirs:
      g_raw_density, g_rgb = ops.composite_bwd(
          lv['ccfg'], lv['raw_density'], lv['tdist'], R.directions, lv['weights'], raw_rgb=lv['raw_rgb'],
          density_noise=lv['dnoise'], bg=lv['bg'], g_rgb_out=g_rgb_out, g_weights=g_weights, want_f32=True,
          exposure_scale=lv['expo'], g_exposure_scale=g_expo if lv['expo'] is not None else None, losses=losses,
          g_x_out=g_x_out)
      g4 = self._buf(('bwd', slot, 'g4'), (M, 4), f32)
      g4[:, 0].copy_(g_raw_density.view(M))
      g4[:, 1:4].copy_(g_rgb.view(M, 3))
      dn, dr = plan.density, plan.rgb
      w4 = self._buf(('bwd', slot, 'w4', W), (W, 4), f32)
      w4[:, 0].copy_(flat[dn.kernel_off:dn.kernel_off + W])
      w4[:, 1:4].copy_(flat[dr.kernel_off:dr.kernel_off + 3 * W].view(W, 3))
      t4 = self._buf(('bwd', slot, 't4', W), (W + 1, 4), f32)
      t4.zero_()
      ops.small_head_bwd(x_last, W, g4, w4, M=M, K=W, Cn=4, dX=dA, lddx=W, relu_mask=relu, dW=t4[:W].view(-1), db=t4[W])
      act_vjp(mlp['zs'][-1] if not relu else None, dA)
      for (d, c0) in plan.head_segs:
        ops.scatter_add(t4, 4, 0, c0, W, d.fan_out, gslice(d.kernel_off, W * d.fan_out), d.fan_out)
        ops.scatter_add(t4, 4, W, c0, 1, d.fan_out, gslice(d.bias_off, d.fan_out), d.fan_out)
    elif plan.has_rgb:
      bw = hp.bottleneck_width
      e = plan.packed['head']
      nh = e['nb_pad']
      dHB = self._buf(('bwd', slot, 'dHB', nh, plan.module_name), (M, nh), bf16, zero=True)
      head_gcol = self._head_gcol(plan)
      assert head_gcol or not panel
      g_den_f32, g_rgb = ops.composite_bwd(
          lv['ccfg'], lv['raw_density'], lv['tdist'], R.directions, lv['weights'], raw_rgb=lv['raw_rgb'],
          density_noise=lv['dnoise'], bg=lv['bg'], g_rgb_out=g_rgb_out, g_weights=g_weights,
          g_den_bf16=dHB.view(-1)[bw:], ld_bf16=nh, want_f32=head_gcol, exposure_scale=lv['expo'],
          g_exposure_scale=g_expo if lv['expo'] is not None else None, losses=losses, g_x_out=g_x_out)
      g_raw_rgb = g_rgb.view(M, 3)
      if head_gcol:
        g_vec = self._buf(('bwd', slot, 'g_den_vec'), (M,), bf16)
        ops.cast_f32_to_bf16(g_den_f32.view(-1), 1, M, 1, g_vec, 1, 0)
        ops.colsum(dHB.view(-1)[bw:], M, 1, gslice(plan.density.bias_off, 1), ld=nh)
      if plan.diffuse_on:
        g_raw_rgb = ops.ref_color_bwd(mlp['raw_rgb_pre'], mlp['small'], hp.rgb_premultiplier, hp.rgb_bias,
                                      hp.rgb_padding, hp.use_specular_tint, g_raw_rgb.contiguous(), dHB, bw + 4, bw + 7)
      WV = hp.net_width_viewdirs
      vacts = mlp['vacts']
      d = plan.rgb
      NV = len(plan.view)
      dV0 = dv_buf(NV - 1, NV)
      h_last = vacts[-1]
      ops.small_head_bwd(h_last, WV, g_raw_rgb, flat[d.kernel_off:d.kernel_off + d.fan_in * 3].view(d.fan_in, 3),
                         M=M, K=WV, Cn=3, dX=dV0, lddx=WV, relu_mask=relu,
                         dW=gslice(d.kernel_off, d.fan_in * 3), db=gslice(d.bias_off, 3))
      act_vjp(mlp['vzs'][-1] if not relu else None, dV0)
      dy = dV0
      VI = mlp['VI']
      dVIa = dVIb = None
      want_glo = plan.glo > 0 and self._glo_cam is not None
      gGa = self._buf(('bwd', slot, 'gGa'), (M, plan.glo), f32) if want_glo else None
      gGb = None
      glo_kw = lambda t: dict(Cf=t, ldcf=plan.glo, f0=plan.glo_col, nf=plan.glo) if want_glo else {}
      for i in reversed(range(len(plan.view))):
        d, concat = plan.view[i]
        e = plan.packed[('view', i)]
        inp = VI if i == 0 else vacts[i - 1]
        in_w = plan.ldVI if i == 0 else WV
        ops.gemm_tn(inp, dy, gslice(d.kernel_off, d.fan_in * d.fan_out), M=M, K=in_w, N=WV,
                    lda=inp.stride(0), ldb=WV, ldc=d.fan_out,
                    k_valid=(plan.vi_width if i == 0 else WV), n_valid=d.fan_out,
                    bias_out=gslice(d.bias_off, d.fan_out), bias_n_valid=d.fan_out)
        if concat:
          ops.gemm_tn(VI, dy, gslice(d.kernel_off + WV * d.fan_out, plan.vi_width * d.fan_out), M=M,
                      K=plan.ldVI, N=WV, lda=plan.ldVI, ldb=WV, ldc=d.fan_out, k_valid=plan.vi_width,
                      n_valid=d.fan_out)
        if concat:
          first_skip = dVIb is None
          tVI = self._buf(('bwd', slot, 'dVIb', 0 if first_skip else 1), (M, plan.ldVI), bf16)
          tG = self._buf(('bwd', slot, 'gGb', 0 if first_skip else 1), (M, plan.glo), f32) if want_glo else None
          B2 = self._w(plan, e['b2_off'], plan.ldVI, e['b_ld'])
          ops.gemm_nt(dy, B2, M=M, N=plan.ldVI, K1=e['b_ld'], Cb=tVI, ldcb=plan.ldVI, nb=plan.ldVI, **glo_kw(tG))
          if first_skip:
            dVIb, gGb = tVI, tG
          else:
            ops.add_cols_bf16(dVIb, tVI, dVIb, plan.ldVI)
            if want_glo:
              gGb.add_(tG)
        Bw = self._w(plan, e['b_off'], e['b_rows'], e['b_ld'])
        if i == 0:
          if plan.ref:
            dVIa = self._buf(('bwd', slot, 'dVIa'), (M, plan.ldVI), bf16)
            ops.gemm_nt(dy, Bw, M=M, N=e['b_rows'], K1=e['b_ld'], Cb=dVIa, ldcb=plan.ldVI, nb=plan.ldVI, **glo_kw(gGa))
          else:
            ops.gemm_nt(dy, Bw, M=M, N=e['b_rows'], K1=e['b_ld'], Cb=dHB, ldcb=nh, nb=bw, **glo_kw(gGa))
        else:
          other = dv_buf(i - 1, NV)
          if relu:
            ops.gemm_nt(dy, Bw, M=M, N=WV, K1=e['b_ld'], mask=vacts[i - 1], ldmask=WV, Cb=other, ldcb=WV, nb=WV)
          else:
            ops.gemm_nt(dy, Bw, M=M, N=WV, K1=e['b_ld'], Cb=other, ldcb=WV, nb=WV)
            act_vjp(mlp['vzs'][i - 1], other)
          dy = other
      if want_glo:
        G = plan.glo
        ops.glo_bwd(gGa, gGb, self._glo_cam, M // n, n, grads[self.glo_off:self.glo_off + self.num_glo_embeddings * G],
                    self.num_glo_embeddings, G)
      if dVIb is not None and not plan.ref:
        ops.add_cols_bf16(dHB, dVIb, dHB, bw)
      if plan.dn and g_normals is not None:
        g_raw_grad = ops.density_normals_bwd(mlp['raw_grad'], g_normals.view(M, 3))
      if plan.pn and g_npred is not None:
        ops.pred_normals_bwd(mlp['small'], 1, g_npred.view(M, 3), dHB, bw + 1)
      if plan.ref:
        g_raw_grad = ops.ref_head_bwd(mlp['small'], mlp.get('raw_grad'), R.viewdirs, n, plan.ide, hp.roughness_bias,
                                      dVIa, dVIb, bw, g_npred, g_normals, dHB, bw + 1, bw + 10, features=plan.features,
                                      deg_view=hp.deg_view)
      e = plan.packed['head']
      if head_gcol:
        db_, dd_ = plan.bottleneck, plan.density
        ops.gemm_tn(x_last, dHB, gslice(db_.kernel_off, W * bw), M=M, K=W, N=bw, lda=W, ldb=nh, ldc=bw,
                    bias_out=gslice(db_.bias_off, bw), bias_n_valid=bw, gcol=g_vec, gcol_out=gslice(dd_.kernel_off, W), **tn_a)
      else:
        tmpW = self._buf(('bwd', slot, 'tmpW', W, nh), (W, nh), f32)
        tmpW.zero_()
        tmpb = self._buf(('bwd', slot, 'tmpb', nh), (nh,), f32)
        tmpb.zero_()
        ops.gemm_tn(x_last, dHB, tmpW, M=M, K=W, N=nh, lda=W, ldb=nh, ldc=nh, bias_out=tmpb,
                    bias_n_valid=plan.head_cols)
        for (d, c0) in plan.head_segs:
          ops.scatter_add(tmpW, nh, 0, c0, W, d.fan_out, gslice(d.kernel_off, W * d.fan_out), d.fan_out)
          ops.scatter_add(tmpb, nh, 0, c0, 1, d.fan_out, gslice(d.bias_off, d.fan_out), d.fan_out)
      Bw = self._w(plan, e['b_off'], _rup(W, 128), e['b_ld'])
      ops.gemm_nt(dHB, Bw, M=M, N=_rup(W, 128), K1=_rup(plan.head_cols, 32 if (panel and _HEAD_K32) else 64), Cb=dA, ldcb=W, nb=W,
                  **mask_kw(len(acts) - 1), **lay_c)
      act_vjp(mlp['zs'][-1] if not relu else None, dA)
    else:
      g_raw_density, _ = ops.composite_bwd(
          lv['ccfg'], lv['raw_density'], lv['tdist'], R.directions, lv['weights'], density_noise=lv['dnoise'],
          bg=lv['bg'], g_rgb_out=g_rgb_out, g_weights=g_weights, want_f32=True, losses=losses, g_x_out=g_x_out)
      d = plan.density
      if mlp.get('chain'):
        w_head = flat[d.kernel_off:d.kernel_off + W]
        ops.small_head_bwd(x_last, W, g_raw_density.view(M, 1), w_head.view(W, 1), M=M, K=W, Cn=1, dX=None,
                           relu_mask=False, dW=gslice(d.kernel_off, W), db=gslice(d.bias_off, 1))
        D = len(plan.trunk)
        r1 = _rank1_last(plan, D, W, g_feat_out is not None)
        dYs = [None if (r1 and i == D - 1) else self._buf(('bwd', slot, 'dYc', W, i, lv['level']), (M, W), bf16) for i in range(D)]
        Bws = [None] + [self._w(plan, plan.packed[('trunk', i)]['b_off'], _rup(W, 128), plan.packed[('trunk', i)]['b_ld'])
                        for i in range(1, D)]
        ops.mlp_chain_bwd(g_raw_density.view(M), w_head, mlp['bits'], Bws, dYs, M=M, W=W)
        feat = lv['feat']
        for i, (dl, concat) in enumerate(plan.trunk):
          inp, in_w, kv = (feat, plan.ldF, plan.F) if i == 0 else (acts[i - 1], W, W)
          ops.gemm_tn(inp, dYs[i], gslice(dl.kernel_off, kv * W), M=M, K=in_w, N=W, lda=in_w, ldb=W, ldc=W,
                      k_valid=kv, n_valid=W, bias_out=gslice(dl.bias_off, W), bias_n_valid=W,
                      rank1=(g_raw_density.view(M), w_head, mlp['bits'][i]) if dYs[i] is None else None)
          if concat:
            ops.gemm_tn(feat, dYs[i], gslice(dl.kernel_off + W * W, plan.F * W), M=M, K=plan.ldF, N=W,
                        lda=plan.ldF, ldb=W, ldc=W, k_valid=plan.F, n_valid=W)
          if i == 0 or concat:
            feat_grad(i, dYs[i])
        return
      ops.small_head_bwd(x_last, W, g_raw_density.view(M, 1), flat[d.kernel_off:d.kernel_off + W].view(W, 1),
                         M=M, K=W, Cn=1, dX=dA, lddx=W, relu_mask=relu,
                         dW=gslice(d.kernel_off, W), db=gslice(d.bias_off, 1))
      act_vjp(mlp['zs'][-1] if not relu else None, dA)
    feat = lv['feat']
    t_extras = None
    if g_raw_grad is not None:
      t_extras = self._tangent_backward(plan, flat, grads, mlp, feat, M, g_raw_grad, slot, g_tfeat_out)
    if mlp.get('chain_trunk'):
      dYs = [self._buf(('bwd', slot, 'dYc', W, i), (M, W), bf16) for i in range(D - 1)] + [None]
      Bws = [None] + [self._w(plan, plan.packed[('trunk', i)]['b_off'], _rup(W, 128), plan.packed[('trunk', i)]['b_ld'])
                      for i in range(1, D)]
      ops.mlp_chain_bwd(None, None, mlp['bits'], Bws, dYs, M=M, W=W, dY_in=dA)
      dYs[D - 1] = dA
      for i, (d, concat) in enumerate(plan.trunk):
        inp, in_w, kv = (feat, plan.ldF, plan.F) if i == 0 else (acts[i - 1], W, W)
        ops.gemm_tn(inp, dYs[i], gslice(d.kernel_off, kv * W), M=M, K=in_w, N=W, lda=in_w, ldb=W, ldc=W,
                    k_valid=kv, n_valid=W, bias_out=gslice(d.bias_off, W), bias_n_valid=W)
        if concat:
          ops.gemm_tn(feat, dYs[i], gslice(d.kernel_off + W * W, plan.F * W), M=M, K=plan.ldF, N=W,
                      lda=plan.ldF, ldb=W, ldc=W, k_valid=plan.F, n_valid=W)
        if i == 0 or concat:
          feat_grad(i, dYs[i])
      return
    dy = dA
    pair = bool(_PAIR_DXDW and panel and self.device.type == 'cuda' and (M // 256) % 8 == 0)
    if pair:
      cur_s = torch.cuda.current_stream(self.device)
      if getattr(self, '_dw_stream', None) is None:
        self._dw_stream = torch.cuda.Stream(device=self.device)
        self._half_cus = max(8, torch.cuda.get_device_properties(self.device).multi_processor_count // 2 // 8 * 8)
        self._pair_events = {}
      dw_done = None

    def pair_event(kind, i):
      ev = self._pair_events.get((kind, i))
      if ev is None:
        ev = self._pair_events[(kind, i)] = torch.cuda.Event()
      return ev

    try:
      for i in reversed(range(len(plan.trunk))):
        d, concat = plan.trunk[i]
        e = plan.packed[('trunk', i)]
        if t_extras is not None:
          ops.add_cols_bf16(dy, t_extras[i], dy, W)
        if pair and i > 0:
          ready = pair_event('ready', i)
          ready.record(cur_s)
          self._dw_stream.wait_event(ready)
          with torch.cuda.stream(self._dw_stream):
            ops.gemm_tn(acts[i - 1], dy, gslice(d.kernel_off, W * W), M=M, K=W, N=W, lda=W, ldb=W, ldc=W,
                        bias_out=gslice(d.bias_off, W), bias_n_valid=W, m_interleave=True, max_wgs=self._half_cus, **tn_a, **tn_b)
            if concat:
              ops.gemm_tn(feat, dy, gslice(d.kernel_off + W * W, plan.F * W), M=M, K=plan.ldF, N=W,
                          lda=plan.ldF, ldb=W, ldc=W, k_valid=plan.F, n_valid=W, **tn_b)
            done = pair_event('done', i)
            done.record(self._dw_stream)
          if concat:
            feat_grad(i, dy, dy_panel=panel)
          if dw_done is not None:
            cur_s.wait_event(dw_done)
          Bw = self._w(plan, e['b_off'], _rup(W, 128), e['b_ld'])
          other = dy_buf(i - 1)
          ops.gemm_nt(dy, Bw, M=M, N=_rup(W, 128), K1=e['b_ld'], Cb=other, ldcb=W, nb=W, max_wgs=self._half_cus,
                      **mask_kw(i - 1), **lay_ac)
          dw_done = done
          dy = other
          continue
        if pair and dw_done is not None:
          cur_s.wait_event(dw_done)
          dw_done = None
        if i == 0:
          ops.gemm_tn(feat, dy, gslice(d.kernel_off, plan.F * W), M=M, K=plan.ldF, N=W, lda=plan.ldF, ldb=W,
                      ldc=W, k_valid=plan.F, n_valid=W, bias_out=gslice(d.bias_off, W), bias_n_valid=W, **tn_b)
        else:
          ops.gemm_tn(acts[i - 1], dy, gslice(d.kernel_off, W * W), M=M, K=W, N=W, lda=W, ldb=W, ldc=W,
                      bias_out=gslice(d.bias_off, W), bias_n_valid=W, **tn_a, **tn_b)
          if concat:
            ops.gemm_tn(feat, dy, gslice(d.kernel_off + W * W, plan.F * W), M=M, K=plan.ldF, N=W,
                        lda=plan.ldF, ldb=W, ldc=W, k_valid=plan.F, n_valid=W, **tn_b)
        if i == 0 or concat:
          feat_grad(i, dy, dy_panel=panel)
        if i > 0:
          Bw = self._w(plan, e['b_off'], _rup(W, 128), e['b_ld'])
          other = dy_buf(i - 1)
          ops.gemm_nt(dy, Bw, M=M, N=_rup(W, 128), K1=e['b_ld'], Cb=other, ldcb=W, nb=W, walk_descending=bool(i & 1),
                      **mask_kw(i - 1), **lay_ac)
          act_vjp(mlp['zs'][i - 1] if not relu else None, other)
          dy = other
    finally:
      if pair and dw_done is not None:
        cur_s.wait_event(dw_done)

  @_in_library
  def backward_prop_levels(self, lvs, flat, grads, g_weights, losses):
    Lg = len(lvs)
    plan: MLPPlan = lvs[0]['plan']
    M, W, D = lvs[0]['M'], plan.W, len(plan.trunk)
    Mall = Lg * M
    R = self._saved['rays']
    g_all = self._buf(('bwd', 'g_props', Lg), (Mall,), f32)
    for k, lv in enumerate(lvs):
      assert lv['group'] == (k, Lg) and lv['M'] == M and lv['plan'] is plan and lv['mlp'].get('chain')
      ops.composite_bwd(lv['ccfg'], lv['raw_density'], lv['tdist'], R.directions, lv['weights'],
                        density_noise=lv['dnoise'], bg=lv['bg'], g_rgb_out=None, g_weights=g_weights[k], want_f32=True,
                        losses=losses[k], g_raw_density_out=g_all[k * M:(k + 1) * M].view(lv['raw_density'].shape))

    def whole(name, cols, dtype):
      return self._buf((('lvl', 'props', Lg), name), (Mall,) + cols, dtype)

    acts = [whole(('act', i), (W,), bf16) for i in range(D)]
    bits = [whole(('bits', i), (W // 8,), torch.uint8) for i in range(D)]
    feat = whole('feat', (plan.ldF,), bf16)
    d = plan.density
    w_head = flat[d.kernel_off:d.kernel_off + W]
    ops.small_head_bwd(acts[-1], W, g_all.view(Mall, 1), w_head.view(W, 1), M=Mall, K=W, Cn=1, dX=None,
                       relu_mask=False, dW=grads[d.kernel_off:d.kernel_off + W], db=grads[d.bias_off:d.bias_off + 1])
    r1 = _rank1_last(plan, D, W, False)
    dYs = [None if (r1 and i == D - 1) else self._buf(('bwd', 'dYc', W, i, 'props'), (Mall, W), bf16) for i in range(D)]
    Bws = [None] + [self._w(plan, plan.packed[('trunk', i)]['b_off'], _rup(W, 128), plan.packed[('trunk', i)]['b_ld'])
                    for i in range(1, D)]
    ops.mlp_chain_bwd(g_all, w_head, bits, Bws, dYs, M=Mall, W=W)
    for i, (dl, concat) in enumerate(plan.trunk):
      inp, in_w, kv = (feat, plan.ldF, plan.F) if i == 0 else (acts[i - 1], W, W)
      ops.gemm_tn(inp, dYs[i], grads[dl.kernel_off:dl.kernel_off + kv * W], M=Mall, K=in_w, N=W, lda=in_w, ldb=W,
                  ldc=W, k_valid=kv, n_valid=W, bias_out=grads[dl.bias_off:dl.bias_off + W], bias_n_valid=W,
                  rank1=(g_all, w_head, bits[i]) if dYs[i] is None else None)
      if concat:
        o = dl.kernel_off + W * W
        ops.gemm_tn(feat, dYs[i], grads[o:o + plan.F * W], M=Mall, K=plan.ldF, N=W, lda=plan.ldF, ldb=W, ldc=W,
                    k_valid=plan.F, n_valid=W)

  def _tangent_backward(self, plan, flat, grads, mlp, feat, M, g_raw_grad, slot, g_tfeat_out=None):
    W = plan.W
    M3 = 3 * M
    T_acts, T_feat, bits = mlp['T_acts'], mlp['T_feat'], mlp['bits']

    def gslice(off, size):
      return grads[off:off + size]

    gA = self._buf(('bwd', slot, 'gTA', W), (M3, W), bf16)
    gB = self._buf(('bwd', slot, 'gTB', W), (M3, W), bf16)
    d = plan.density
    relu = plan.hp.net_activation == 'relu'
    extras = None if relu else [self._buf(('bwd', slot, 'T_extra', W, i), (M, W), bf16) for i in range(len(plan.trunk))]
    ops.small_head_bwd(T_acts[-1], W, g_raw_grad.view(M3, 1), flat[d.kernel_off:d.kernel_off + W].view(W, 1),
                       M=M3, K=W, Cn=1, dX=gA, lddx=W, relu_mask=False, dW=gslice(d.kernel_off, W), db=None,
                       bits=bits[-1] if relu else None, bits_row_mod=M if relu else 0)
    gy, other = gA, gB
    D = len(plan.trunk)
    Gs = None
    if _TANGENT_CHAIN and relu and D >= 2 and self._chain_ok(plan) and all(b is not None for b in bits):
      Gs = [self._buf(('bwd', slot, 'gT', W, i), (M3, W), bf16) for i in range(D - 1)] + [gA]
      Bws = [None] + [self._w(plan, plan.packed[('trunk', i)]['b_off'], _rup(W, 128), plan.packed[('trunk', i)]['b_ld'])
                      for i in range(1, D)]
      for c in range(3):
        rows = slice(c * M, (c + 1) * M)
        ops.mlp_chain_bwd(None, None, bits, Bws, [g[rows] for g in Gs[:-1]] + [None], M=M, W=W, dY_in=gA[rows])
    for i in reversed(range(len(plan.trunk))):
      d, concat = plan.trunk[i]
      e = plan.packed[('trunk', i)]
      if Gs is not None:
        gy = Gs[i]
      if not relu:
        ops.act_tangent_bwd(plan.hp.net_activation, mlp['zs'][i], mlp['T_pre'][i], gy, extras[i])
      if g_tfeat_out is not None and (i == 0 or concat):
        gT = self._buf(('bwd', slot, 'g_tfeat', len(g_tfeat_out)), (M3, plan.ldF), bf16)
        ops.gemm_nt(gy, self._w(plan, e['bf_off'], plan.ldF, e['bf_ld']), M=M3, N=plan.ldF, K1=e['bf_ld'], Cb=gT, ldcb=plan.ldF,
                    nb=plan.ldF)
        g_tfeat_out.append(gT)
      if i == 0:
        ops.gemm_tn(T_feat, gy, gslice(d.kernel_off, plan.F * W), M=M3, K=plan.ldF, N=W, lda=plan.ldF, ldb=W,
                    ldc=W, k_valid=plan.F, n_valid=W)
      else:
        ops.gemm_tn(T_acts[i - 1], gy, gslice(d.kernel_off, W * W), M=M3, K=W, N=W, lda=W, ldb=W, ldc=W)
        if concat:
          ops.gemm_tn(T_feat, gy, gslice(d.kernel_off + W * W, plan.F * W), M=M3, K=plan.ldF, N=W,
                      lda=plan.ldF, ldb=W, ldc=W, k_valid=plan.F, n_valid=W)
        if Gs is None:
          Bw = self._w(plan, e['b_off'], _rup(W, 128), e['b_ld'])
          ops.gemm_nt(gy, Bw, M=M3, N=_rup(W, 128), K1=e['b_ld'], Cb=other, ldcb=W, nb=W,
                      **(dict(bits_in=bits[i - 1], bits_row_mod=M) if relu else {}))
          gy, other = other, gy
    return extras




def construct_model(rng, rays, config, device='cuda'):
  model = Model(config=config)
  model.build(device)
  flat = model.init_flat_params(seed=0 if rng is None else int(rng))
  variables = {'flat': flat, 'params': model.params_tree(flat)}
  model.bind(variables)
  return model, variables


def render_image(render_fn, rays, rng, config, verbose=True, world_size=1, rank=0):
  height, width = rays.origins.shape[:2]
  num_rays = height * width
  rays = rays.map(lambda r: r.reshape((num_rays, -1)))
  chunks = []
  idx0s = range(0, num_rays, config.render_chunk_size)
  for i_chunk, idx0 in enumerate(idx0s):
    if verbose and i_chunk % max(1, len(idx0s) // 10) == 0:
# ... 35 lines not shown
```

### multinerf_amd/ops.py

```python

import ctypes as C
import os

import torch

from multinerf_amd import _lib as L

bf16 = torch.bfloat16
f32 = torch.float32


def _ptr(t):
  return None if t is None else C.c_void_p(t.data_ptr())


def _stream():
  return C.c_void_p(torch.cuda.current_stream().cuda_stream)


def _on_device(t):
  return t.is_cuda


def act_dtype():
# ... 411 lines not shown
  a.C, a.ldc = Cout.data_ptr(), ldc if ldc else Cout.stride(0)
  a.k_valid = K if k_valid is None else k_valid
  a.n_valid = N if n_valid is None else n_valid
  a.bias_out = bias_out.data_ptr() if bias_out is not None else None
  a.bias_n_valid = bias_n_valid
  a.gcol = gcol.data_ptr() if gcol is not None else None
  a.gcol_out = gcol_out.data_ptr() if gcol_out is not None else None
  a.a_layout, a.b_layout = a_layout, b_layout
  a.m_interleave, a.max_wgs = int(bool(m_interleave)), int(max_wgs)
  _e = PROFILE.start()
  L.check(lib().mnr_gemm_tn_bf16(C.byref(a), _stream()))
  PROFILE.stop(_e)


def mlp_chain_fwd(feat, K0, layers, *, M, W, w_head=None, b_head=None, head_out=None, acts=None, bits=None, skip_layer=0):
  depth = len(layers)
  if not 1 <= depth <= L.CHAIN_MAX_DEPTH:
    raise ValueError(f'mlp_chain_fwd: depth {depth}')
  _chk(feat, bf16, 'feat')
  _chk(w_head, bf16, 'w_head', allow_none=True)
  _chk(b_head, f32, 'b_head', allow_none=True)
  _chk(head_out, f32, 'head_out', allow_none=True)
  a = L.MlpChainFwdArgs()
  a.M, a.W, a.depth, a.skip_layer = M, W, depth, int(skip_layer)
  a.feat, a.ld_feat, a.K0 = feat.data_ptr(), feat.stride(0), K0
  for i, (Bt, bias) in enumerate(layers):
    _chk(Bt, bf16, f'Bt[{i}]')
    _chk(bias, f32, f'bias[{i}]')
    assert Bt.shape[0] >= W and bias.numel() == W
    a.Bt[i], a.ldb[i], a.bias[i] = Bt.data_ptr(), Bt.stride(0), bias.data_ptr()
    if acts is not None and acts[i] is not None:
      _chk(acts[i], bf16, f'acts[{i}]')
      assert acts[i].shape == (M, W)
      a.acts[i] = acts[i].data_ptr()
    if bits is not None and bits[i] is not None:
      _chk(bits[i], torch.uint8, f'bits[{i}]')
      assert bits[i].shape == (M, W // 8)
      a.bits[i] = bits[i].data_ptr()
  if w_head is not None:
    assert w_head.numel() >= W and head_out is not None and head_out.numel() == M
    a.w_head, a.head_out = w_head.data_ptr(), head_out.data_ptr()
    a.b_head = b_head.data_ptr() if b_head is not None else None
  _e = PROFILE.start()
  L.check(lib().mnr_mlp_chain_fwd(C.byref(a), _stream()))
  PROFILE.stop(_e)


def mlp_chain_fwd_ipe(tdist, origins, directions, radii, basis, layers, *, M, W, ray_shape, warp_contract, min_deg,
                      max_deg, disable_integration=False, w_head=None, b_head=None, head_out=None, act_last=None):
  depth = len(layers)
  if not 1 <= depth <= L.CHAIN_MAX_DEPTH:
    raise ValueError(f'mlp_chain_fwd_ipe: depth {depth}')
  for x, nm in ((tdist, 'tdist'), (origins, 'origins'), (directions, 'directions'), (radii, 'radii'), (basis, 'basis')):
    _chk(x, f32, nm)
  _chk(w_head, bf16, 'w_head', allow_none=True)
  _chk(b_head, f32, 'b_head', allow_none=True)
  _chk(head_out, f32, 'head_out', allow_none=True)
  B, n1 = tdist.shape
  assert B * (n1 - 1) == M and origins.shape[0] == B and directions.shape[0] == B and radii.numel() == B
  a = L.MlpChainFwdArgs()
  a.M, a.W, a.depth, a.skip_layer = M, W, depth, 0
  for i, (Bt, bias) in enumerate(layers):
    _chk(Bt, bf16, f'Bt[{i}]')
    _chk(bias, f32, f'bias[{i}]')
    assert Bt.shape[0] >= W and bias.numel() == W
    a.Bt[i], a.ldb[i], a.bias[i] = Bt.data_ptr(), Bt.stride(0), bias.data_ptr()
  if act_last is not None:
    _chk(act_last, bf16, 'act_last')
    assert act_last.shape == (M, W)
    a.acts[depth - 1] = act_last.data_ptr()
  if w_head is not None:
    assert w_head.numel() >= W and head_out is not None and head_out.numel() == M
    a.w_head, a.head_out = w_head.data_ptr(), head_out.data_ptr()
    a.b_head = b_head.data_ptr() if b_head is not None else None
  q = L.ChainIpeArgs()
  q.cfg = _ipe_cfg(ray_shape, warp_contract, disable_integration, basis, min_deg, max_deg)
  q.n = n1 - 1
  q.tdist, q.origins, q.directions, q.radii, q.basis = _ptr(tdist), _ptr(origins), _ptr(directions), _ptr(radii), _ptr(basis)
  _e = PROFILE.start()
  L.check(lib().mnr_mlp_chain_fwd_ipe(C.byref(a), C.byref(q), _stream()))
  PROFILE.stop(_e)


def mlp_chain_bwd(g_head, w_head, bits, Bws, dYs, *, M, W, dY_in=None):
  depth = len(bits)
  assert len(dYs) == depth and len(Bws) == depth
  a = L.MlpChainBwdArgs()
  a.M, a.W, a.depth = M, W, depth
  if dY_in is not None:
    _chk(dY_in, bf16, 'dY_in')
    assert dY_in.shape == (M, W) and dYs[depth - 1] is None
    a.dY_in = dY_in.data_ptr()
  else:
    _chk(g_head, f32, 'g_head')
    _chk(w_head, f32, 'w_head')
    assert g_head.numel() == M and w_head.numel() == W
    a.g_head, a.w_head = g_head.data_ptr(), w_head.data_ptr()
  for i in range(depth):
    _chk(bits[i], torch.uint8, f'bits[{i}]')
    assert bits[i].shape == (M, W // 8)
    a.bits[i] = bits[i].data_ptr()
    if dYs[i] is not None:
      _chk(dYs[i], bf16, f'dY[{i}]')
      assert dYs[i].shape == (M, W)
      a.dY[i] = dYs[i].data_ptr()
    if i >= 1:
      _chk(Bws[i], bf16, f'Bw[{i}]')
      a.Bw[i], a.ldb[i] = Bws[i].data_ptr(), Bws[i].stride(0)
  _e = PROFILE.start()
  L.check(lib().mnr_mlp_chain_bwd(C.byref(a), _stream()))
  PROFILE.stop(_e)


def colsum(X, M, n_valid, out, ld=None):
  _chk(X, bf16, 'X')
  _chk(out, f32, 'out')
  L.check(lib().mnr_colsum_bf16(_ptr(X), ld if ld else X.stride(0), M, n_valid, _ptr(out), _stream()))


def pack_weights(params, descs_dev, n_desc, max_elems, dst):
  _chk(params, f32, 'params')
  _chk(dst, bf16, 'dst')
  L.check(lib().mnr_pack_weights_bf16(_ptr(params), _ptr(descs_dev), n_desc, max_elems, _ptr(dst), _stream()))


def scatter_add(src, ld_src, row0, col0, rows, cols, dst, ld_dst):
  _chk(src, f32, 'src')
  _chk(dst, f32, 'dst')
  L.check(lib().mnr_scatter_add_f32(_ptr(src), ld_src, row0, col0, rows, cols, _ptr(dst), ld_dst, _stream()))


def cast_f32_to_bf16(src, ld_src, M, n, dst, ld_dst, col0):
  _chk(src, f32, 'src')
  _chk(dst, bf16, 'dst')
  L.check(lib().mnr_cast_f32_to_bf16(_ptr(src), ld_src, M, n, _ptr(dst), ld_dst, col0, _stream()))


def act_fwd(kind, z, a):
  _chk(z, bf16, 'z')
  _chk(a, bf16, 'a')
  assert z.shape == a.shape
  L.check(lib().mnr_act_fwd_bf16(L.NET_ACT[kind], z.numel(), _ptr(z), _ptr(a), _stream()))


def act_bwd(kind, z, d):
  _chk(z, bf16, 'z')
  _chk(d, bf16, 'd')
  assert z.shape == d.shape
  L.check(lib().mnr_act_bwd_bf16(L.NET_ACT[kind], z.numel(), _ptr(z), _ptr(d), _stream()))


def act_tangent_fwd(kind, z, U, T):
  for x, nm in ((z, 'z'), (U, 'U'), (T, 'T')):
    _chk(x, bf16, nm)
  assert U.shape == T.shape and U.numel() == 3 * z.numel()
  L.check(lib().mnr_act_tangent_fwd_bf16(L.NET_ACT[kind], z.numel(), _ptr(z), _ptr(U), _ptr(T), _stream()))


def act_tangent_bwd(kind, z, U, G, extra):
  for x, nm in ((z, 'z'), (U, 'U'), (G, 'G'), (extra, 'extra')):
    _chk(x, bf16, nm)
  assert U.shape == G.shape and U.numel() == 3 * z.numel() and extra.shape == z.shape
  L.check(lib().mnr_act_tangent_bwd_bf16(L.NET_ACT[kind], z.numel(), _ptr(z), _ptr(U), _ptr(G), _ptr(extra), _stream()))


def add_noise_bf16(X, cols, noise, scale):
  _chk(noise, f32, 'noise')
  if X.dtype != act_dtype() or not _on_device(X):
    raise ValueError(f'X must be a {act_dtype()} device tensor')
  M = X.shape[0]
  assert noise.shape == (M, cols)
  L.check(lib().mnr_add_noise_bf16(M, cols, _ptr(X), X.stride(0), _ptr(noise), float(scale), _stream()))


_HEAD_SCRATCH = {}


def _head_scratch(device):
  key = (device, getattr(_stream(), 'value', None))
  t = _HEAD_SCRATCH.get(key)
  if t is None:
    t = _HEAD_SCRATCH[key] = torch.empty(1 << 20, dtype=f32, device=device)
  return t


def small_head_bwd(H, ldh, g, W, *, M, K, Cn, dX=None, lddx=0, relu_mask=True, dW=None, db=None, bits=None,
                   bits_row_mod=0):
  _chk(bits, torch.uint8, 'bits', allow_none=True)
  _chk(H, bf16, 'H')
  _chk(g, f32, 'g')
  _chk(W, f32, 'W')
  _e = PROFILE.start()
  scratch = _head_scratch(H.device)
  L.check(lib().mnr_small_head_bwd(M, K, Cn, _ptr(H), ldh, _ptr(g), _ptr(W), _ptr(dX), lddx, int(relu_mask),
                                   _ptr(dW), _ptr(db), _ptr(bits), bits.stride(0) if bits is not None else 0,
                                   bits_row_mod, _ptr(scratch), scratch.numel(), _stream()))
  PROFILE.stop(_e, 'small_head_bwd', 2 * M * K * (2 if dX is not None else 1) + 4 * M * Cn)




def composite_cfg(n, *, opaque_background, density_act, density_bias, density_noise_std, has_rgb, rgb_act,
                  rgb_premultiplier, rgb_bias, rgb_padding, bg_mode, bg_value):
  return L.CompositeCfg(n, int(opaque_background), L.ACT[density_act], float(density_bias),
                        float(density_noise_std), int(has_rgb), L.ACT[rgb_act], float(rgb_premultiplier),
                        float(rgb_bias), float(rgb_padding), int(bg_mode), float(bg_value))


def composite_fwd(cfg, raw_density, tdist, dirs, *, raw_rgb=None, density_noise=None, bg=None,
                  exposure_scale=None, want_acc=True):
  _chk(raw_density, f32, 'raw_density')
  _chk(tdist, f32, 'tdist')
  _chk(dirs, f32, 'dirs')
  for x, nm in ((raw_rgb, 'raw_rgb'), (density_noise, 'density_noise'), (bg, 'bg'),
                (exposure_scale, 'exposure_scale')):
    _chk(x, f32, nm, allow_none=True)
  B, n = raw_density.shape
  dev = raw_density.device
  density = torch.empty((B, n), dtype=f32, device=dev)
  weights = torch.empty((B, n), dtype=f32, device=dev)
  rgb = torch.empty((B, n, 3), dtype=f32, device=dev) if cfg.has_rgb else None
  rgb_out = torch.empty((B, 3), dtype=f32, device=dev)
  acc = torch.empty((B,), dtype=f32, device=dev) if want_acc else None
  _e = PROFILE.start()
  L.check(lib().mnr_composite_fwd(C.byref(cfg), B, _ptr(raw_density), _ptr(density_noise), _ptr(raw_rgb),
                                  _ptr(tdist), _ptr(dirs), _ptr(bg), _ptr(exposure_scale), _ptr(density),
                                  _ptr(rgb), _ptr(weights), _ptr(rgb_out), _ptr(acc), _stream()))
  PROFILE.stop(_e, 'composite_fwd', 4 * (raw_density.numel() * (2 + 2 + (6 if raw_rgb is not None else 0))))
  return density, rgb, weights, rgb_out, acc


def composite_bwd(cfg, raw_density, tdist, dirs, weights, *, raw_rgb=None, density_noise=None, bg=None,
                  exposure_scale=None, g_rgb_out=None, g_weights=None, g_den_bf16=None, ld_bf16=0,
                  want_f32=True, g_exposure_scale=None, losses=None, g_raw_density_out=None, g_x_out=None):
  B, n = raw_density.shape
  dev = raw_density.device
  for x, nm in ((raw_density, 'raw_density'), (tdist, 'tdist'), (dirs, 'dirs'), (weights, 'weights')):
    _chk(x, f32, nm)
  for x, nm in ((g_rgb_out, 'g_rgb_out'), (g_weights, 'g_weights')):
    _chk(x, f32, nm, allow_none=True)
  _chk(g_den_bf16, bf16, 'g_den_bf16', allow_none=True)
  if g_raw_density_out is not None:
    _chk(g_raw_density_out, f32, 'g_raw_density_out')
    assert want_f32 and g_raw_density_out.shape == (B, n) and g_raw_density_out.is_contiguous()
    g_raw_density = g_raw_density_out
  else:
    g_raw_density = torch.empty((B, n), dtype=f32, device=dev) if want_f32 else None
  g_raw_rgb = torch.empty((B, n, 3), dtype=f32, device=dev) if cfg.has_rgb else None
  a = L.LevelBwdArgs()
  a.cfg = cfg
  a.B = B
  a.B_valid = B if losses is None else int(losses['B_valid'])
  p = lambda t: None if t is None else t.data_ptr()
  a.raw_density, a.density_noise, a.raw_rgb, a.tdist, a.dirs = p(raw_density), p(density_noise), p(raw_rgb), p(tdist), p(dirs)
  a.bg, a.exposure_scale, a.weights, a.g_rgb_out, a.g_weights = p(bg), p(exposure_scale), p(weights), p(g_rgb_out), p(g_weights)
  a.g_raw_density, a.g_raw_density_bf16, a.ld_bf16 = p(g_raw_density), p(g_den_bf16), ld_bf16
  a.g_raw_rgb, a.g_exposure_scale = p(g_raw_rgb), p(g_exposure_scale)
  a.data_loss_type, a.wloss_mode = -1, 0
  if g_x_out is not None:
    _chk(g_x_out, f32, 'g_x_out')
    assert g_x_out.shape == (B, n) and g_x_out.is_contiguous()
    a.g_x = p(g_x_out)
  keep = []
  if losses is not None and losses.get('data') is not None:
    d = losses['data']
    if d['type'] not in L.DATA_LOSS:
      raise ValueError(f"unsupported data_loss_type {d['type']!r}")
    for k in ('rgb_out', 'gt', 'lossmult', 'denom', 'stats'):
      _chk(d[k], f32, 'data.' + k)
    assert d['rgb_out'].shape[0] == B and d['gt'].shape[0] == B and d['lossmult'].shape[0] == B
    a.data_loss_type, a.charb_padding, a.data_loss_mult = L.DATA_LOSS[d['type']], float(d['charb_padding']), float(d['mult'])
    a.rgb_out, a.gt, a.lossmult, a.lm_c = p(d['rgb_out']), p(d['gt']), p(d['lossmult']), d['lossmult'].shape[-1]
    a.denom, a.data_stats = p(d['denom']), p(d['stats'])
    keep.append(d)
  if losses is not None and losses.get('weights') is not None:
    w = losses['weights']
    _chk(w['sdist'], f32, 'weights.sdist')
    _chk(w['stat'], f32, 'weights.stat')
    assert w['sdist'].shape == (B, n + 1)
    a.wloss_mult, a.sdist, a.wloss_stat = float(w['mult']), p(w['sdist']), p(w['stat'])
    if w['mode'] == 'interlevel':
      _chk(w['t_ref'], f32, 'weights.t_ref')
      _chk(w['w_ref'], f32, 'weights.w_ref')
      assert w['t_ref'].shape[0] == B and w['t_ref'].shape[1] == w['w_ref'].shape[1] + 1
      a.wloss_mode, a.n_ref, a.t_ref, a.w_ref = 1, w['w_ref'].shape[1], p(w['t_ref']), p(w['w_ref'])
    elif w['mode'] == 'distortion':
      a.wloss_mode = 2
    else:
      raise ValueError(f"weights.mode {w['mode']!r}")
    keep.append(w)
  _e = PROFILE.start()
  L.check(lib().mnr_level_bwd(C.byref(a), _stream()))
  PROFILE.stop(_e, 'composite_bwd', 4 * (raw_density.numel() * (3 + (3 if raw_rgb is not None else 0))) + (2 + (12 if raw_rgb is not None else 0)) * raw_density.numel())
  return g_raw_density, g_raw_rgb


def exposure_scale(exposure_values, exposure_idx, offsets):
  _chk(exposure_values, f32, 'exposure_values')
  _chk(exposure_idx, torch.int32, 'exposure_idx')
  _chk(offsets, f32, 'offsets', allow_none=True)
  B = exposure_values.numel()
  out = torch.empty((B, 3), dtype=f32, device=exposure_values.device)
  L.check(lib().mnr_exposure_scale(B, _ptr(exposure_values), _ptr(exposure_idx), _ptr(offsets), _ptr(out), _stream()))
  return out


def exposure_scale_bwd(exposure_values, exposure_idx, g_scale, g_offsets, B_valid):
  _chk(g_scale, f32, 'g_scale')
  _chk(g_offsets, f32, 'g_offsets')
  L.check(lib().mnr_exposure_scale_bwd(B_valid, _ptr(exposure_values), _ptr(exposure_idx), _ptr(g_scale),
                                       _ptr(g_offsets), _stream()))


def render_extras(weights, tdist, t_far):
  for x, nm in ((weights, 'weights'), (tdist, 'tdist'), (t_far, 't_far')):
    _chk(x, f32, nm)
  B, n = weights.shape
  out = torch.empty((B, 4), dtype=f32, device=weights.device)
  L.check(lib().mnr_render_extras(B, n, _ptr(weights), _ptr(tdist), _ptr(t_far), _ptr(out), _stream()))
  return out




class IdeTablesDev:

  def __init__(self, deg_view, device):
    from multinerf_amd import ref_utils
    m, l, mat, sigma = ref_utils.ide_tables(deg_view)
    self.T = len(m)
    self.m = torch.as_tensor(m, dtype=torch.int32, device=device)
    self.l = torch.as_tensor(l, dtype=torch.int32, device=device)
    self.mat = torch.as_tensor(mat, dtype=f32, device=device).contiguous()
    self.sigma = torch.as_tensor(sigma, dtype=f32, device=device)
    self.c = L.IdeTables(self.T, mat.shape[0] - 1, self.m.data_ptr(), self.l.data_ptr(), self.sigma.data_ptr(),
                         self.mat.data_ptr())


REF_PRED_NORMALS, REF_DENSITY_NORMALS, REF_REFLECT, REF_IDE, REF_N_DOT_V, REF_ROUGHNESS = 1, 2, 4, 8, 16, 32
REF_ALL = 63

# ... 454 lines not shown
```

### multinerf_amd/streams.py

```python

import os

import torch


class BackwardStreams:

  def __init__(self, device):
    self.device = torch.device(device)
    self.prop = torch.cuda.Stream(device=self.device)

  @staticmethod
  def from_env(device):
    if os.environ.get('MNR_SIDE_STREAM', '1') == '0':
      return None
    return BackwardStreams(device)


def describe_env():
  return {'side_stream': os.environ.get('MNR_SIDE_STREAM', '1') != '0'}
```

Measured before the change: 535,400.

## Fuse density head weight/bias gradients into chain backward and composite backward kernels

```diff
diff --git a/include/mnerf.h b/include/mnerf.h
--- a/include/mnerf.h
+++ b/include/mnerf.h
@@ -165,6 +165,14 @@
 int mnr_mlp_chain_bwd(const mnr_mlp_chain_bwd_args* args, void* stream);
 
 typedef struct {
+  const uint16_t* x_last; int ldx;
+  float* dw_out;
+  float* db_out;
+  float* scratch; int64_t scratch_floats;
+} mnr_chain_head_grad_args;
+int mnr_mlp_chain_bwd_head(const mnr_mlp_chain_bwd_args* args, const mnr_chain_head_grad_args* head, void* stream);
+
+typedef struct {
   const uint16_t* A; int lda; int K;
   const uint16_t* B; int ldb; int N;
   int64_t M;
@@ -250,6 +258,8 @@
   const float* rgb_out; const float* gt; const float* lossmult; int lm_c; const float* denom; float* data_stats;
   int wloss_mode; float wloss_mult; const float* sdist; int n_ref; const float* t_ref; const float* w_ref; float* wloss_stat;
   float* g_x;
+  uint16_t* g_density_vec;
+  float* db_density;
 } mnr_level_bwd_args;
 int mnr_level_bwd(const mnr_level_bwd_args* args, void* stream);
 
diff --git a/multinerf_amd/_lib.py b/multinerf_amd/_lib.py
--- a/multinerf_amd/_lib.py
+++ b/multinerf_amd/_lib.py
@@ -7,7 +7,7 @@
 LIB_PATH = os.environ.get('MNR_LIB_PATH') or os.path.join(HERE, 'libmnerf_hip.so')
 LIB_F32_PATH = os.path.join(HERE, 'libmnerf_hip_f32.so')
 HEADER_PATH = os.path.join(os.path.dirname(HERE), 'include', 'mnerf.h')
-F32_ABSENT = ('mnr_mlp_chain_fwd', 'mnr_mlp_chain_fwd_ipe', 'mnr_mlp_chain_bwd')
+F32_ABSENT = ('mnr_mlp_chain_fwd', 'mnr_mlp_chain_fwd_ipe', 'mnr_mlp_chain_bwd', 'mnr_mlp_chain_bwd_head')
 
 
 def describe():
@@ -97,6 +97,10 @@
               ('dY', vp * CHAIN_MAX_DEPTH), ('dY_in', vp)]
 
 
+class ChainHeadGradArgs(C.Structure):
+  _fields_ = [('x_last', vp), ('ldx', C.c_int), ('dw_out', vp), ('db_out', vp), ('scratch', vp), ('scratch_floats', C.c_int64)]
+
+
 class PackDesc(C.Structure):
   _fields_ = [('src_off', C.c_int64), ('rows_in', C.c_int), ('cols_out', C.c_int),
               ('dst_off', C.c_int64), ('ld', C.c_int), ('row0', C.c_int), ('col0', C.c_int),
@@ -119,7 +123,7 @@
               ('data_loss_type', C.c_int), ('charb_padding', C.c_float), ('data_loss_mult', C.c_float),
               ('rgb_out', vp), ('gt', vp), ('lossmult', vp), ('lm_c', C.c_int), ('denom', vp), ('data_stats', vp),
               ('wloss_mode', C.c_int), ('wloss_mult', C.c_float), ('sdist', vp), ('n_ref', C.c_int), ('t_ref', vp),
-              ('w_ref', vp), ('wloss_stat', vp), ('g_x', vp)]
+              ('w_ref', vp), ('wloss_stat', vp), ('g_x', vp), ('g_density_vec', vp), ('db_density', vp)]
 
 
 class SdistBwdArgs(C.Structure):
@@ -208,6 +212,7 @@
     'mnr_gemm_tn_bf16': ([C.POINTER(GemmTNArgs), vp], i32),
     'mnr_mlp_chain_fwd': ([C.POINTER(MlpChainFwdArgs), vp], i32),
     'mnr_mlp_chain_bwd': ([C.POINTER(MlpChainBwdArgs), vp], i32),
+    'mnr_mlp_chain_bwd_head': ([C.POINTER(MlpChainBwdArgs), C.POINTER(ChainHeadGradArgs), vp], i32),
     'mnr_mlp_chain_fwd_ipe': ([C.POINTER(MlpChainFwdArgs), C.POINTER(ChainIpeArgs), vp], i32),
     'mnr_colsum_bf16': ([vp, i32, i64, i32, vp, vp], i32),
     'mnr_pack_weights_bf16': ([vp, vp, i32, i32, vp, vp], i32),
diff --git a/multinerf_amd/csrc/common.h b/multinerf_amd/csrc/common.h
--- a/multinerf_amd/csrc/common.h
+++ b/multinerf_amd/csrc/common.h
@@ -52,6 +52,8 @@
   } while (0)
 
 static inline int mnr_cdiv(long long a, long long b) { return (int)((a + b - 1) / b); }
+
+int small_head_reduce_launch(int nblk, int n, int n_dw, const float* partials, float* dW, float* db, void* stream);
 
 static inline int mnr_cu_count() {
   static int cus = 0;
diff --git a/multinerf_amd/csrc/fused_mlp.hip b/multinerf_amd/csrc/fused_mlp.hip
--- a/multinerf_amd/csrc/fused_mlp.hip
+++ b/multinerf_amd/csrc/fused_mlp.hip
@@ -441,14 +441,79 @@
   }
 }
 
+template <int W, bool HG>
+__device__ __forceinline__ void fm_rank1_start(char* smem, const mnr_mlp_chain_bwd_args& p, const mnr_chain_head_grad_args& hg,
+                                               int tid, int64_t m0) {
+  typedef FmCfg<W> C;
+  const int last = p.depth - 1;
+  const int t_ = fm_opaque(tid);
+  const int row0 = t_ / C::CPR, ch = t_ % C::CPR;
+  float wh[8];
+  {
+    const f32x4 a = *(const f32x4*)(p.w_head + ch * 8), b = *(const f32x4*)(p.w_head + ch * 8 + 4);
+#pragma unroll
+    for (int e = 0; e < 4; ++e) wh[e] = a[e], wh[4 + e] = b[e];
+  }
+  char* lptr = smem + (ch >> 3) * FM_KT_BYTES + row0 * 128 + (((ch & 7) ^ ((row0 >> 1) & 7)) << 4);
+  const int64_t ro = m0 + row0;
+  const uint8_t* bl = p.bits[last] + ro * (W / 8) + (ch & ~3);
+  const float* gp = p.g_head + ro;
+  bf16* dst = p.dY[last] ? (bf16*)p.dY[last] + ro * W + ch * 8 : nullptr;
+  float g[C::COPY_ITERS];
+  unsigned mb[C::COPY_ITERS];
+#pragma unroll
+  for (int u = 0; u < C::COPY_ITERS; ++u) {
+    g[u] = gp[u * C::ROW_STEP];
+    mb[u] = *(const unsigned*)(bl + (int64_t)u * C::ROW_STEP * (W / 8)) >> ((ch & 3) * 8);
+  }
+  bf16x8 xv[HG ? C::COPY_ITERS : 1];
+  if (HG) {
+    const bf16* xp = (const bf16*)hg.x_last + ro * hg.ldx + ch * 8;
+    __builtin_amdgcn_sched_barrier(0);
+#pragma unroll
+    for (int u = 0; u < C::COPY_ITERS; ++u) xv[u] = *(const bf16x8*)(xp + (int64_t)u * C::ROW_STEP * hg.ldx);
+    __builtin_amdgcn_sched_barrier(0);
+  }
+#pragma unroll
+  for (int u = 0; u < C::COPY_ITERS; ++u) {
+    bf16x8 v;
+#pragma unroll
+    for (int e = 0; e < 8; ++e) v[e] = (bf16)(((mb[u] >> e) & 1u) ? g[u] * wh[e] : 0.0f);
+    *(bf16x8*)(lptr + u * C::ROW_STEP * 128) = v;
+    if (dst) *(bf16x8*)(dst + (int64_t)u * C::ROW_STEP * W) = v;
+  }
+  if (HG) {
+    float hd[8] = {0.0f, 0.0f, 0.0f, 0.0f, 0.0f, 0.0f, 0.0f, 0.0f};
+    float sg = 0.0f;
+#pragma unroll
+    for (int u = 0; u < C::COPY_ITERS; ++u) {
+#pragma unroll
+      for (int e = 0; e < 8; ++e) hd[e] += g[u] * (float)xv[u][e];
+      sg += g[u];
+    }
+    float* hs = (float*)(smem + C::BIAS_OFF) + t_;
+#pragma unroll
+    for (int e = 0; e < 8; ++e) hs[e * 512] += hd[e];
+    if (ch == 0) hs[8 * 512] += sg;
+  }
+}
+
+#define FM_HG_SLOTS 9
 template <int W>
-__global__ __launch_bounds__(512) void mlp_chain_bwd_kernel(mnr_mlp_chain_bwd_args p, int defer) {
+__global__ __launch_bounds__(512) void mlp_chain_bwd_kernel(mnr_mlp_chain_bwd_args p, int defer, mnr_chain_head_grad_args hg) {
   typedef FmCfg<W> C;
   extern __shared__ __attribute__((aligned(16))) char smem[];
+  static_assert(C::LDS_BYTES - C::BIAS_OFF >= FM_HG_SLOTS * 512 * 4, "head-gradient slots");
   const int tid = threadIdx.x, lane = tid & 63;
   const int wave = __builtin_amdgcn_readfirstlane(tid >> 6);
   const int cw = wave % C::NW, rg = wave / C::NW;
   const int64_t tiles = p.M / FM_ROWS;
+  const bool hg_on = hg.x_last != nullptr;
+  if (hg_on) {
+    float* hs = (float*)(smem + C::BIAS_OFF) + fm_opaque(tid);
+#pragma unroll
+    for (int k = 0; k < FM_HG_SLOTS; ++k) hs[k * 512] = 0.0f;
+  }
 
   for (int64_t tile = blockIdx.x; tile < tiles; tile += gridDim.x) {
     const int64_t m0 = tile * FM_ROWS;
@@ -464,35 +529,8 @@
       MNR_GPU_ONLY(asm volatile("s_waitcnt vmcnt(0)" ::: "memory"));
       MNR_SIM_HOOK(hipsim::wait_vmcnt(0));
     } else {
-      const int last = p.depth - 1;
-      const int t_ = fm_opaque(tid);
-      const int row0 = t_ / C::CPR, ch = t_ % C::CPR;
-      float wh[8];
-      {
-        const f32x4 a = *(const f32x4*)(p.w_head + ch * 8), b = *(const f32x4*)(p.w_head + ch * 8 + 4);
-#pragma unroll
-        for (int e = 0; e < 4; ++e) wh[e] = a[e], wh[4 + e] = b[e];
-      }
-      char* lptr = smem + (ch >> 3) * FM_KT_BYTES + row0 * 128 + (((ch & 7) ^ ((row0 >> 1) & 7)) << 4);
-      const int64_t ro = m0 + row0;
-      const uint8_t* bl = p.bits[last] + ro * (W / 8) + (ch & ~3);
-      const float* gp = p.g_head + ro;
-      bf16* dst = p.dY[last] ? (bf16*)p.dY[last] + ro * W + ch * 8 : nullptr;
-      float g[C::COPY_ITERS];
-      unsigned mb[C::COPY_ITERS];
-#pragma unroll
-      for (int u = 0; u < C::COPY_ITERS; ++u) {
-        g[u] = gp[u * C::ROW_STEP];
-        mb[u] = *(const unsigned*)(bl + (int64_t)u * C::ROW_STEP * (W / 8)) >> ((ch & 3) * 8);
-      }
-#pragma unroll
-      for (int u = 0; u < C::COPY_ITERS; ++u) {
-        bf16x8 v;
-#pragma unroll
-        for (int e = 0; e < 8; ++e) v[e] = (bf16)(((mb[u] >> e) & 1u) ? g[u] * wh[e] : 0.0f);
-        *(bf16x8*)(lptr + u * C::ROW_STEP * 128) = v;
-        if (dst) *(bf16x8*)(dst + (int64_t)u * C::ROW_STEP * W) = v;
-      }
+      if (hg_on) fm_rank1_start<W, true>(smem, p, hg, tid, m0);
+      else fm_rank1_start<W, false>(smem, p, hg, tid, m0);
     }
     bf16x8 w0[FM_WCHUNK];
     if (p.depth > 1) {
@@ -525,6 +563,16 @@
       FM_STAMP(4 + 3 * li);
     }
     if (tl_on) g_fm_timeline[32 * (int64_t)blockIdx.x + 31] = __builtin_amdgcn_s_memrealtime();
+  }
+  if (hg_on) {
+    __syncthreads();
+    const int j = fm_opaque(tid);
+    if (j <= W) {
+      const float* hs = (const float*)(smem + C::BIAS_OFF) + (j < W ? (j & 7) * 512 + (j >> 3) : 8 * 512);
+      float sum = 0.0f;
+      for (int i = 0; i < 512 / C::CPR; ++i) sum += hs[i * C::CPR];
+      hg.scratch[(int64_t)blockIdx.x * (W + 1) + j] = sum;
+    }
   }
 }
 
@@ -582,30 +630,49 @@
   return MNR_OK;
 }
 
-extern "C" int mnr_mlp_chain_bwd(const mnr_mlp_chain_bwd_args* a, void* stream) {
-  MNR_CHECK_ARG(a != nullptr, "mnr_mlp_chain_bwd: null args");
-  if (int s = fm_check_common("mnr_mlp_chain_bwd", a->M, a->W, a->depth)) return s;
+static int fm_chain_bwd_launch(const char* who, const mnr_mlp_chain_bwd_args* a, const mnr_chain_head_grad_args* h, void* stream) {
+  MNR_CHECK_ARG(a != nullptr, "%s: null args", who);
+  if (int s = fm_check_common(who, a->M, a->W, a->depth)) return s;
   MNR_CHECK_ARG(a->dY_in ? ((uintptr_t)a->dY_in % 16) == 0 : (a->g_head && a->w_head && ((uintptr_t)a->w_head % 16) == 0),
-                "mnr_mlp_chain_bwd: needs dY_in (16-byte aligned) or a head gradient with a 16-byte-aligned head kernel");
+                "%s: needs dY_in (16-byte aligned) or a head gradient with a 16-byte-aligned head kernel", who);
   for (int i = 0; i < a->depth; ++i) {
-    MNR_CHECK_ARG(a->bits[i] && ((uintptr_t)a->bits[i] % 4) == 0, "mnr_mlp_chain_bwd: layer %d needs its ReLU mask bits", i);
-    MNR_CHECK_ARG(a->dY[i] || i == a->depth - 1, "mnr_mlp_chain_bwd: dY[%d] missing", i);
-    MNR_CHECK_ARG(!(a->dY_in && i == a->depth - 1 && a->dY[i]), "mnr_mlp_chain_bwd: with dY_in the last dY is the input itself");
-    MNR_CHECK_ARG(!a->dY[i] || ((uintptr_t)a->dY[i] % 16) == 0, "mnr_mlp_chain_bwd: dY[%d] must be 16-byte aligned", i);
+    MNR_CHECK_ARG(a->bits[i] && ((uintptr_t)a->bits[i] % 4) == 0, "%s: layer %d needs its ReLU mask bits", who, i);
+    MNR_CHECK_ARG(a->dY[i] || i == a->depth - 1, "%s: dY[%d] missing", who, i);
+    MNR_CHECK_ARG(!(a->dY_in && i == a->depth - 1 && a->dY[i]), "%s: with dY_in the last dY is the input itself", who);
+    MNR_CHECK_ARG(!a->dY[i] || ((uintptr_t)a->dY[i] % 16) == 0, "%s: dY[%d] must be 16-byte aligned", who, i);
     if (i >= 1)
       MNR_CHECK_ARG(a->Bw[i] && a->ldb[i] % 8 == 0 && a->ldb[i] >= a->W && ((uintptr_t)a->Bw[i] % 16) == 0,
-                    "mnr_mlp_chain_bwd: layer %d operand", i);
+                    "%s: layer %d operand", who, i);
   }
   const int grid = fm_grid(a->M / FM_ROWS);
+  mnr_chain_head_grad_args hg = {};
+  if (h) {
+    MNR_CHECK_ARG(!a->dY_in && a->g_head && a->w_head, "%s: the head gradient needs g_head / w_head (no dY_in)", who);
+    MNR_CHECK_ARG(h->x_last && ((uintptr_t)h->x_last % 16) == 0 && h->ldx % 8 == 0 && h->ldx >= a->W,
+                  "%s: x_last must be 16-byte aligned with ldx %% 8 == 0 and ldx >= W", who);
+    MNR_CHECK_ARG(h->dw_out && h->scratch && h->scratch_floats >= (int64_t)grid * (a->W + 1),
+                  "%s: needs dw_out and a scratch of grid * (W + 1) = %lld floats", who, (long long)grid * (a->W + 1));
+    hg = *h;
+  }
   if (a->W == 256) {
     (void)hipFuncSetAttribute((const void*)mlp_chain_bwd_kernel<256>, hipFuncAttributeMaxDynamicSharedMemorySize, FmCfg<256>::LDS_BYTES);
-    hipLaunchKernelGGL(mlp_chain_bwd_kernel<256>, dim3(grid), dim3(512), FmCfg<256>::LDS_BYTES, (hipStream_t)stream, *a, g_fm_defer);
+    hipLaunchKernelGGL(mlp_chain_bwd_kernel<256>, dim3(grid), dim3(512), FmCfg<256>::LDS_BYTES, (hipStream_t)stream, *a, g_fm_defer, hg);
   } else {
     (void)hipFuncSetAttribute((const void*)mlp_chain_bwd_kernel<128>, hipFuncAttributeMaxDynamicSharedMemorySize, FmCfg<128>::LDS_BYTES);
-    hipLaunchKernelGGL(mlp_chain_bwd_kernel<128>, dim3(grid), dim3(512), FmCfg<128>::LDS_BYTES, (hipStream_t)stream, *a, g_fm_defer);
+    hipLaunchKernelGGL(mlp_chain_bwd_kernel<128>, dim3(grid), dim3(512), FmCfg<128>::LDS_BYTES, (hipStream_t)stream, *a, g_fm_defer, hg);
   }
   MNR_CHECK_LAUNCH();
+  if (h) return small_head_reduce_launch(grid, a->W + 1, a->W, hg.scratch, hg.dw_out, hg.db_out, stream);
   return MNR_OK;
+}
+
+extern "C" int mnr_mlp_chain_bwd(const mnr_mlp_chain_bwd_args* a, void* stream) {
+  return fm_chain_bwd_launch("mnr_mlp_chain_bwd", a, nullptr, stream);
+}
+
+extern "C" int mnr_mlp_chain_bwd_head(const mnr_mlp_chain_bwd_args* a, const mnr_chain_head_grad_args* h, void* stream) {
+  MNR_CHECK_ARG(h != nullptr, "mnr_mlp_chain_bwd_head: null head-gradient args");
+  return fm_chain_bwd_launch("mnr_mlp_chain_bwd_head", a, h, stream);
 }
 
 #pragma clang fp contract(off)
diff --git a/multinerf_amd/csrc/gemm.hip b/multinerf_amd/csrc/gemm.hip
--- a/multinerf_amd/csrc/gemm.hip
+++ b/multinerf_amd/csrc/gemm.hip
@@ -920,6 +920,13 @@
   }
 }
 
+int small_head_reduce_launch(int nblk, int n, int n_dw, const float* partials, float* dW, float* db, void* stream) {
+  hipLaunchKernelGGL(small_head_reduce_kernel, dim3(mnr_cdiv(n, 128), 16), dim3(128), 0, (hipStream_t)stream, nblk, n, n_dw,
+                     partials, dW, db);
+  MNR_CHECK_LAUNCH();
+  return MNR_OK;
+}
+
 extern "C" int mnr_small_head_bwd(int64_t M, int K, int C, const uint16_t* H, int ldh, const float* g,
                                   const float* W, uint16_t* dX, int lddx, int apply_relu_mask, float* dW,
                                   float* db, const uint8_t* mask_bits, int ld_bits, int64_t bits_row_mod,
@@ -945,10 +952,7 @@
                      (bf16*)dX, lddx, apply_relu_mask, dW, db, rows_per_block, mask_bits, ld_bits, bits_row_mod, partials);
   MNR_CHECK_LAUNCH();
   if (partials) {
-    const int n = K * C + C;
-    hipLaunchKernelGGL(small_head_reduce_kernel, dim3(mnr_cdiv(n, 128), 16), dim3(128), 0, (hipStream_t)stream, grid, n,
-                       K * C, partials, dW, db);
-    MNR_CHECK_LAUNCH();
-  }
-  return MNR_OK;
-}
+    return small_head_reduce_launch(grid, K * C + C, K * C, partials, dW, db, stream);
+  }
+  return MNR_OK;
+}
diff --git a/multinerf_amd/csrc/render.hip b/multinerf_amd/csrc/render.hip
--- a/multinerf_amd/csrc/render.hip
+++ b/multinerf_amd/csrc/render.hip
@@ -331,11 +331,20 @@
   }
   __syncthreads();
   if (a.g_raw_density) cp_store_rows(l_den, a.g_raw_density + ray0 * n, rows, n, S);
-  if (a.g_raw_density_bf16) {
+  if (a.g_raw_density_bf16 || a.g_density_vec || a.db_density) {
     bf16* gb = (bf16*)a.g_raw_density_bf16;
+    bf16* gv = (bf16*)a.g_density_vec;
+    float s_db = 0.0f;
     for (int e = threadIdx.x; e < rows * n; e += CP_THREADS) {
       const int rr = e / n, i = e % n;
-      gb[(ray0 * n + e) * (int64_t)a.ld_bf16] = (bf16)l_den[i * S + rr];
+      const bf16 v = (bf16)l_den[i * S + rr];
+      if (gb) gb[(ray0 * n + e) * (int64_t)a.ld_bf16] = v;
+      if (gv) gv[ray0 * n + e] = v;
+      s_db += (float)v;
+    }
+    if (a.db_density) {
+      s_db = ls_wave_sum(s_db);
+      if (threadIdx.x == 0) unsafeAtomicAdd(a.db_density, s_db);
     }
   }
   if (c.has_rgb && a.g_raw_rgb) cp_store_rows(l_rgb, a.g_raw_rgb + ray0 * n * 3, rows, 3 * n, S);
@@ -645,11 +654,20 @@
     }
   };
   if (a.g_raw_density) store_rows(L.den, a.g_raw_density + ray0 * n, n);
-  if (a.g_raw_density_bf16) {
+  if (a.g_raw_density_bf16 || a.g_density_vec || a.db_density) {
     bf16* gb = (bf16*)a.g_raw_density_bf16;
+    bf16* gv = (bf16*)a.g_density_vec;
+    float s_db = 0.0f;
     for (int e = threadIdx.x; e < rows * n; e += CP_THREADS) {
       const int rr = e / n, i = e - rr * n;
-      gb[(ray0 * n + e) * (int64_t)a.ld_bf16] = (bf16)lds[rr * L.stride + L.den + i];
+      const bf16 v = (bf16)lds[rr * L.stride + L.den + i];
+      if (gb) gb[(ray0 * n + e) * (int64_t)a.ld_bf16] = v;
+      if (gv) gv[ray0 * n + e] = v;
+      s_db += (float)v;
+    }
+    if (a.db_density) {
+      s_db = ls_wave_sum(s_db);
+      if (threadIdx.x == 0) unsafeAtomicAdd(a.db_density, s_db);
     }
   }
   if (c.has_rgb && a.g_raw_rgb) store_rows(L.rgb, a.g_raw_rgb + ray0 * n * 3, 3 * n);
@@ -760,7 +778,7 @@
   MNR_CHECK_ARG(a->B > 0 && a->B_valid > 0 && a->B_valid <= a->B && a->raw_density && a->tdist && a->dirs && a->weights,
                 "mnr_level_bwd: null argument");
   MNR_CHECK_ARG(cfg->n >= 1 && cfg->n <= 1024, "mnr_level_bwd: n out of range");
-  MNR_CHECK_ARG(a->g_raw_density || a->g_raw_density_bf16, "mnr_level_bwd: no density-gradient output");
+  MNR_CHECK_ARG(a->g_raw_density || a->g_raw_density_bf16 || a->g_density_vec, "mnr_level_bwd: no density-gradient output");
   MNR_CHECK_ARG(!cfg->has_rgb || a->raw_rgb, "mnr_level_bwd: has_rgb needs raw_rgb");
   MNR_CHECK_ARG(cfg->bg_mode == 0 || a->bg, "mnr_level_bwd: bg_mode 1 needs bg");
   MNR_CHECK_ARG(a->data_loss_type < 0 || (a->data_loss_type <= MNR_LOSS_RAWNERF && a->rgb_out && a->gt && a->lossmult &&
diff --git a/multinerf_amd/models.py b/multinerf_amd/models.py
--- a/multinerf_amd/models.py
+++ b/multinerf_amd/models.py
@@ -11,6 +11,7 @@
 from multinerf_amd import geopoly
 from multinerf_amd import gin
 from multinerf_amd import ops
+from multinerf_amd import streams
 from multinerf_amd import utils
 
 F32_EPS = float(np.finfo(np.float32).eps)
@@ -49,6 +50,7 @@
 _PAIR_DXDW = True
 _TANGENT_CHAIN = True
 _HEAD_K32 = True
+_FUSED_HEAD_GRAD, _FUSED_LEVEL_GRAD = streams.fused_head_grad_from_env()
 
 
 
@@ -1225,13 +1227,16 @@
       dHB = self._buf(('bwd', slot, 'dHB', nh, plan.module_name), (M, nh), bf16, zero=True)
       head_gcol = self._head_gcol(plan)
       assert head_gcol or not panel
+      vjp_vec = head_gcol and _FUSED_LEVEL_GRAD
+      g_vec = self._buf(('bwd', slot, 'g_den_vec'), (M,), bf16) if vjp_vec else None
       g_den_f32, g_rgb = ops.composite_bwd(
           lv['ccfg'], lv['raw_density'], lv['tdist'], R.directions, lv['weights'], raw_rgb=lv['raw_rgb'],
           density_noise=lv['dnoise'], bg=lv['bg'], g_rgb_out=g_rgb_out, g_weights=g_weights,
-          g_den_bf16=dHB.view(-1)[bw:], ld_bf16=nh, want_f32=head_gcol, exposure_scale=lv['expo'],
-          g_exposure_scale=g_expo if lv['expo'] is not None else None, losses=losses, g_x_out=g_x_out)
+          g_den_bf16=dHB.view(-1)[bw:], ld_bf16=nh, want_f32=head_gcol and not vjp_vec, exposure_scale=lv['expo'],
+          g_exposure_scale=g_expo if lv['expo'] is not None else None, losses=losses, g_x_out=g_x_out,
+          g_den_vec=g_vec, db_density=gslice(plan.density.bias_off, 1) if vjp_vec else None)
       g_raw_rgb = g_rgb.view(M, 3)
-      if head_gcol:
+      if head_gcol and not vjp_vec:
         g_vec = self._buf(('bwd', slot, 'g_den_vec'), (M,), bf16)
         ops.cast_f32_to_bf16(g_den_f32.view(-1), 1, M, 1, g_vec, 1, 0)
         ops.colsum(dHB.view(-1)[bw:], M, 1, gslice(plan.density.bias_off, 1), ld=nh)
@@ -1335,14 +1340,16 @@
       d = plan.density
       if mlp.get('chain'):
         w_head = flat[d.kernel_off:d.kernel_off + W]
-        ops.small_head_bwd(x_last, W, g_raw_density.view(M, 1), w_head.view(W, 1), M=M, K=W, Cn=1, dX=None,
-                           relu_mask=False, dW=gslice(d.kernel_off, W), db=gslice(d.bias_off, 1))
+        head_grad = (x_last, gslice(d.kernel_off, W), gslice(d.bias_off, 1)) if _FUSED_HEAD_GRAD else None
+        if head_grad is None:
+          ops.small_head_bwd(x_last, W, g_raw_density.view(M, 1), w_head.view(W, 1), M=M, K=W, Cn=1, dX=None,
+                             relu_mask=False, dW=gslice(d.kernel_off, W), db=gslice(d.bias_off, 1))
         D = len(plan.trunk)
         r1 = _rank1_last(plan, D, W, g_feat_out is not None)
         dYs = [None if (r1 and i == D - 1) else self._buf(('bwd', slot, 'dYc', W, i, lv['level']), (M, W), bf16) for i in range(D)]
         Bws = [None] + [self._w(plan, plan.packed[('trunk', i)]['b_off'], _rup(W, 128), plan.packed[('trunk', i)]['b_ld'])
                         for i in range(1, D)]
-        ops.mlp_chain_bwd(g_raw_density.view(M), w_head, mlp['bits'], Bws, dYs, M=M, W=W)
+        ops.mlp_chain_bwd(g_raw_density.view(M), w_head, mlp['bits'], Bws, dYs, M=M, W=W, head_grad=head_grad)
         feat = lv['feat']
         for i, (dl, concat) in enumerate(plan.trunk):
           inp, in_w, kv = (feat, plan.ldF, plan.F) if i == 0 else (acts[i - 1], W, W)
@@ -1471,13 +1478,15 @@
     feat = whole('feat', (plan.ldF,), bf16)
     d = plan.density
     w_head = flat[d.kernel_off:d.kernel_off + W]
-    ops.small_head_bwd(acts[-1], W, g_all.view(Mall, 1), w_head.view(W, 1), M=Mall, K=W, Cn=1, dX=None,
-                       relu_mask=False, dW=grads[d.kernel_off:d.kernel_off + W], db=grads[d.bias_off:d.bias_off + 1])
+    head_grad = (acts[-1], grads[d.kernel_off:d.kernel_off + W], grads[d.bias_off:d.bias_off + 1]) if _FUSED_HEAD_GRAD else None
+    if head_grad is None:
+      ops.small_head_bwd(acts[-1], W, g_all.view(Mall, 1), w_head.view(W, 1), M=Mall, K=W, Cn=1, dX=None,
+                         relu_mask=False, dW=grads[d.kernel_off:d.kernel_off + W], db=grads[d.bias_off:d.bias_off + 1])
     r1 = _rank1_last(plan, D, W, False)
     dYs = [None if (r1 and i == D - 1) else self._buf(('bwd', 'dYc', W, i, 'props'), (Mall, W), bf16) for i in range(D)]
     Bws = [None] + [self._w(plan, plan.packed[('trunk', i)]['b_off'], _rup(W, 128), plan.packed[('trunk', i)]['b_ld'])
                     for i in range(1, D)]
-    ops.mlp_chain_bwd(g_all, w_head, bits, Bws, dYs, M=Mall, W=W)
+    ops.mlp_chain_bwd(g_all, w_head, bits, Bws, dYs, M=Mall, W=W, head_grad=head_grad)
     for i, (dl, concat) in enumerate(plan.trunk):
       inp, in_w, kv = (feat, plan.ldF, plan.F) if i == 0 else (acts[i - 1], W, W)
       ops.gemm_tn(inp, dYs[i], grads[dl.kernel_off:dl.kernel_off + kv * W], M=Mall, K=in_w, N=W, lda=in_w, ldb=W,
diff --git a/multinerf_amd/ops.py b/multinerf_amd/ops.py
--- a/multinerf_amd/ops.py
+++ b/multinerf_amd/ops.py
@@ -517,7 +517,7 @@
   PROFILE.stop(_e)
 
 
-def mlp_chain_bwd(g_head, w_head, bits, Bws, dYs, *, M, W, dY_in=None):
+def mlp_chain_bwd(g_head, w_head, bits, Bws, dYs, *, M, W, dY_in=None, head_grad=None):
   depth = len(bits)
   assert len(dYs) == depth and len(Bws) == depth
   a = L.MlpChainBwdArgs()
@@ -542,6 +542,18 @@
     if i >= 1:
       _chk(Bws[i], bf16, f'Bw[{i}]')
       a.Bw[i], a.ldb[i] = Bws[i].data_ptr(), Bws[i].stride(0)
+  if head_grad is not None:
+    x_last, dW, db = head_grad
+    _chk(x_last, bf16, 'x_last')
+    _chk(dW, f32, 'dW')
+    _chk(db, f32, 'db', allow_none=True)
+    assert dY_in is None and x_last.shape == (M, W) and x_last.stride(1) == 1 and dW.numel() == W
+    scratch = _head_scratch(x_last.device)
+    h = L.ChainHeadGradArgs(_ptr(x_last), x_last.stride(0), _ptr(dW), _ptr(db), _ptr(scratch), scratch.numel())
+    _e = PROFILE.start()
+    L.check(lib().mnr_mlp_chain_bwd_head(C.byref(a), C.byref(h), _stream()))
+    PROFILE.stop(_e)
+    return
   _e = PROFILE.start()
   L.check(lib().mnr_mlp_chain_bwd(C.byref(a), _stream()))
   PROFILE.stop(_e)
@@ -667,7 +679,8 @@
 
 def composite_bwd(cfg, raw_density, tdist, dirs, weights, *, raw_rgb=None, density_noise=None, bg=None,
                   exposure_scale=None, g_rgb_out=None, g_weights=None, g_den_bf16=None, ld_bf16=0,
-                  want_f32=True, g_exposure_scale=None, losses=None, g_raw_density_out=None, g_x_out=None):
+                  want_f32=True, g_exposure_scale=None, losses=None, g_raw_density_out=None, g_x_out=None,
+                  g_den_vec=None, db_density=None):
   B, n = raw_density.shape
   dev = raw_density.device
   for x, nm in ((raw_density, 'raw_density'), (tdist, 'tdist'), (dirs, 'dirs'), (weights, 'weights')):
@@ -692,6 +705,13 @@
   a.g_raw_density, a.g_raw_density_bf16, a.ld_bf16 = p(g_raw_density), p(g_den_bf16), ld_bf16
   a.g_raw_rgb, a.g_exposure_scale = p(g_raw_rgb), p(g_exposure_scale)
   a.data_loss_type, a.wloss_mode = -1, 0
+  if g_den_vec is not None:
+    _chk(g_den_vec, bf16, 'g_den_vec')
+    assert g_den_vec.numel() == B * n
+    a.g_density_vec = p(g_den_vec)
+  if db_density is not None:
+    _chk(db_density, f32, 'db_density')
+    a.db_density = p(db_density)
   if g_x_out is not None:
     _chk(g_x_out, f32, 'g_x_out')
     assert g_x_out.shape == (B, n) and g_x_out.is_contiguous()
diff --git a/multinerf_amd/streams.py b/multinerf_amd/streams.py
--- a/multinerf_amd/streams.py
+++ b/multinerf_amd/streams.py
@@ -17,5 +17,12 @@
     return BackwardStreams(device)
 
 
+def fused_head_grad_from_env():
+  v = os.environ.get('MNR_FUSED_HEAD_GRAD', '1')
+  if v not in ('0', '1', 'chain', 'level'):
+    raise ValueError(f'MNR_FUSED_HEAD_GRAD={v!r}: 0, 1, chain or level')
+  return v in ('1', 'chain'), v in ('1', 'level')
+
+
 def describe_env():
-  return {'side_stream': os.environ.get('MNR_SIDE_STREAM', '1') != '0'}
+  return {'side_stream': os.environ.get('MNR_SIDE_STREAM', '1') != '0', 'fused_head_grad': os.environ.get('MNR_FUSED_HEAD_GRAD', '1')}
```

After: 539,100 (median of 6 runs). About the same (+0.7%).
